# KTC-Security-Circle/3d-matching

Hardware: AMD Instinct MI355X
Metric: ICP iterations/sec + RANSAC hypotheses/sec, 100k↔100k pts, 1/2/4/8 GPU (higher is better)
Workload: dtype fp16-split MFMA NN screen + fp32 scan, exact fp64 NN decision, fp64 terms/solve; 1 GPU; cfg1: 100000<->100000 synthetic pair per GPU, 50 point-to-plane ICP iterations, brute-force NN (r=0.12), 1 GPU; ns=100000, nt_per_gpu=100000, parallelism=single, comm=none, comm_ranks=1

## Files before the change

### 3d-matching_amd/csrc/api.cpp

```cpp
#include <cfloat>
#include <chrono>
#include <hip/hip_runtime.h>
#include <string.h>

#include <algorithm>
#include <cmath>
#include <string>
#include <memory>
#include <mutex>
#include <unordered_map>
#include <vector>

#include "linalg.h"
#include "m3d_internal.h"
#include "ddmath.h"

using namespace m3d;

int m3d_fail(m3d_ctx* ctx, int code, const std::string& msg) {
  if (ctx) ctx->err = msg;
  return code;
}

KTimer::KTimer(m3d_ctx* c, int kid, hipStream_t s) : ctx(c), id(kid), st(s) {
// ... 1080 lines not shown
  for (Grid* g : c->grids) {
    grid_free(g);
    delete g;
  }
  for (auto& m : c->morton) {
    if (m.second->refs > 0)
      m.second->orphan = true;
    else
      m3d_cloud_destroy(m.second);
  }
  for (void** p : {reinterpret_cast<void**>(&c->slot), reinterpret_cast<void**>(&c->xyz64),
                   reinterpret_cast<void**>(&c->nrm64), reinterpret_cast<void**>(&c->xyz32)})
    if (in_block(*p, c->block, c->block_bytes)) *p = nullptr;
  block_release(c->block);
  hipFree(c->slot);
  hipFree(c->xyz64);
  hipFree(c->nrm64);
  hipFree(c->xyz32);
  block_release(c->rec64);
  delete c;
}

int64_t m3d_cloud_size(const m3d_cloud* c) { return c ? c->n : -1; }

namespace {
int ensure_grid(m3d_ctx* ctx, const m3d_cloud* c, double cell, hipStream_t st, const Grid** out) {
  for (Grid* g : c->grids)
    if (g->cell_req == cell && g->n_pts == c->n) {
      *out = g;
      return M3D_OK;
    }
  Grid* g = new Grid();
  float lohi[6];
  for (int k = 0; k < 3; ++k) {
    lohi[k] = c->lo[k];
    lohi[3 + k] = c->hi[k];
  }
  hipError_t e = grid_build(c->xyz32, c->n, cell, st, g, &ctx->tmp, c->has_bounds ? lohi : nullptr);
  if (e != hipSuccess) {
    grid_free(g);
    delete g;
    return m3d_fail(ctx, M3D_ERR_HIP, std::string("grid build: ") + hipGetErrorString(e));
  }
  g->cell_req = cell;
  c->grids.push_back(g);
  *out = g;
  return M3D_OK;
}

int ensure_morton_source(m3d_ctx* ctx, const m3d_cloud* c, double cell, const m3d_cloud** out,
                         const Grid** gout) {
  for (auto& m : c->morton)
    if (m.first == cell && m.second->n == c->n) {
      *out = m.second;
      *gout = m.second->grids.front();
      return M3D_OK;
    }
  m3d_cloud* mc = new m3d_cloud();
  mc->ctx = ctx;
  mc->ctx_id = ctx->id;
  Grid* g = new Grid();
  mc->grids.push_back(g);
  hipError_t e = morton_source(c, cell, mc, g, &ctx->tmp, nullptr);
  if (e != hipSuccess) {
    m3d_cloud_destroy(mc);
    return m3d_fail(ctx, M3D_ERR_HIP, std::string("morton source: ") + hipGetErrorString(e));
  }
  c->morton.emplace_back(cell, mc);
  constexpr size_t kMortonKeep = 4;
  for (size_t k = 0; c->morton.size() > kMortonKeep && k + 1 < c->morton.size();) {
    if (c->morton[k].second->refs == 0) {
      m3d_cloud_destroy(c->morton[k].second);
      c->morton.erase(c->morton.begin() + (ptrdiff_t)k);
    } else {
      ++k;
    }
  }
  *out = mc;
  *gout = g;
  return M3D_OK;
}

hipError_t enqueue_nn(m3d_icp* s, int64_t off, hipStream_t st, bool self_seed = false, int64_t q0 = 0,
                      int64_t q1 = -1) {
  m3d_ctx* ctx = s->ctx;
  const bool whole = q0 == 0 && (q1 < 0 || q1 == s->src->n);
  const bool seeded = self_seed && s->keys_clean && off == 0 && whole;
  s->keys_clean = false;
  if (s->params.nn_method == M3D_NN_GRID) {
    KTimer kt(ctx, M3D_KERNEL_NN, st);
    return launch_grid_nn(s->src->xyz32, s->src->n, s->sgrid, s->tgrid, off, s->state, s->keys,
                          s->near2, s->corr, s->dprev, s->tgt->xyz32, s->tgt->n, st, q0, q1,
                          s->hlist, s->hcnt, s->cand_cap, s->pcd64, s->tgt->xyz64, s->hcap, s->scan_xchunk);
  }
  if (!seeded) {
    hipError_t e = launch_icp_keyinit(s, off, st, q0, q1);
    if (e != hipSuccess) return e;
  }
  KTimer kt(ctx, M3D_KERNEL_NN, st);
  return launch_icp_nn(s, off, seeded, st, q0, q1);
}
}

extern "C++" {
namespace m3d {
int icp_shard_nn_range(m3d_icp* s, int64_t off, int64_t q0, int64_t q1, int64_t* dkeys, hipStream_t st) {
  hipError_t e = enqueue_nn(s, off, st, false, q0, q1);
  if (e == hipSuccess) e = launch_shard_winner(s, off, dkeys, st, q0, q1);
  if (e != hipSuccess) return m3d_fail(s->ctx, M3D_ERR_HIP, std::string("shard NN: ") + hipGetErrorString(e));
  return M3D_OK;
}
}
}

namespace {
int icp_create(m3d_ctx* ctx, const m3d_cloud* src, const m3d_cloud* tgt, double max_dist,
               const m3d_icp_params* params, m3d_icp** out, bool run_arena);
}

int m3d_icp_create(m3d_ctx* ctx, const m3d_cloud* src, const m3d_cloud* tgt, double max_dist,
                   const m3d_icp_params* params, m3d_icp** out) {
  return icp_create(ctx, src, tgt, max_dist, params, out, false);
}

namespace {
int32_t heavy_cap(const m3d_icp_params* params, int64_t coarse_max_occ) {
  constexpr int64_t kHeavyCell = 256;
  constexpr int32_t kHeavyCand = 256;
  static const int heavy_env = [] {
    const char* e = getenv("M3D_GRID_HEAVY");
    return e ? std::max(0, atoi(e)) : -1;
  }();
  if (params->nn_method != M3D_NN_GRID) return 0;
  return heavy_env > 0 ? heavy_env : (heavy_env < 0 && coarse_max_occ >= kHeavyCell ? kHeavyCand : 0);
}

int icp_create(m3d_ctx* ctx, const m3d_cloud* src, const m3d_cloud* tgt, double max_dist,
               const m3d_icp_params* params, m3d_icp** out, bool run_arena) {
  if (!ctx) return M3D_ERR_INVALID;
  CHECK_ARG(ctx, src && tgt && params && out, "invalid arguments");
  CHECK_ARG(ctx, max_dist > 0.0, "Invalid max_correspondence_distance.");
  CHECK_ARG(ctx, params->estimation == M3D_EST_POINT_TO_PLANE ||
                     params->estimation == M3D_EST_POINT_TO_POINT,
            "unknown estimation");
  CHECK_ARG(ctx, params->estimation != M3D_EST_POINT_TO_PLANE || tgt->nrm64 != nullptr || tgt->n == 0,
            "TransformationEstimationPointToPlane requires pre-computed normal vectors for target "
            "PointCloud.");
  CHECK_ARG(ctx, params->max_iteration >= 0, "max_iteration must be >= 0");
  CHECK_ARG(ctx, params->nn_method == M3D_NN_BRUTE || params->nn_method == M3D_NN_GRID,
            "unknown nn_method");
  hipSetDevice(ctx->device);
  const Grid *tg = nullptr, *sg = nullptr;
  const m3d_cloud* src_m = nullptr;
  int64_t coarse_max_occ = 0;
  int32_t cand_cap = 0;
  m3d_icp* s = new m3d_icp();
  {
    const double cell = max_dist * 1.001;
    int grc = ensure_grid(ctx, tgt, cell, nullptr, &tg);
    const m3d_cloud* ms = nullptr;
    if (!grc) grc = ensure_morton_source(ctx, src, cell, &ms, &sg);
    if (!grc) src_m = ms;
    if (!grc) {
      hipError_t e = ensure_target_rec(tgt, nullptr);
      if (e != hipSuccess) grc = m3d_fail(ctx, M3D_ERR_HIP, std::string("target records: ") + hipGetErrorString(e));
    }
    if (!grc && params->nn_method == M3D_NN_GRID) {
      hipError_t e = pin_ensure(ctx) == M3D_OK ? hipSuccess : hipErrorOutOfMemory;
      if (e == hipSuccess)
        e = grid_occupancy(const_cast<Grid*>(tg), &ctx->tmp, nullptr, pin_read<unsigned long long>(ctx, true),
                           pin_read<unsigned long long>(ctx, false));
      if (e != hipSuccess) grc = m3d_fail(ctx, M3D_ERR_HIP, std::string("grid occupancy: ") + hipGetErrorString(e));
    }
    if (!grc && params->nn_method == M3D_NN_GRID && tg->n_occ > 0) {
      coarse_max_occ = tg->max_occ;
      const double m = (double)tg->n_pts / (double)tg->n_occ;
      const int div = std::min(4, std::max(1, (int)std::floor(std::sqrt(m / 3.5))));
      if (div > 1) grc = ensure_grid(ctx, tgt, cell / div, nullptr, &tg);
    }
    if (!grc) {
      hipError_t e = build_grid_pts64(tgt, const_cast<Grid*>(tg), nullptr);
      if (e != hipSuccess) grc = m3d_fail(ctx, M3D_ERR_HIP, std::string("grid fp64 points: ") + hipGetErrorString(e));
    }
    if (!grc && params->nn_method == M3D_NN_BRUTE && tg->mf16 == nullptr) {
      hipError_t e = build_mfma_tiles(tgt, const_cast<Grid*>(tg), &ctx->tmp, nullptr);
      if (e != hipSuccess) grc = m3d_fail(ctx, M3D_ERR_HIP, std::string("mfma tiles: ") + hipGetErrorString(e));
    }
    if (!grc) {
      cand_cap = heavy_cap(params, coarse_max_occ);
      const size_t n1 = (size_t)std::max<int64_t>(src->n, 1);
      Carve cv;
      cv.add(&s->state, 1);
      if (params->nn_method == M3D_NN_BRUTE) nn_plan_shape(src->n, &s->nn_qblocks, &s->nn_budget);
      if (s->nn_qblocks > 0) {
        cv.add(&s->nn_cnt, (size_t)s->nn_qblocks);
        cv.add(&s->nn_seen, (size_t)s->nn_qblocks);
        cv.add(&s->nn_table, (size_t)s->nn_budget);
      }
      cv.add(&s->keys, n1);
      cv.add(&s->near2, n1);
      cv.add(&s->dprev, n1);
      cv.add(&s->ld64, n1);
      cv.add(&s->lidx, n1);
      cv.add(&s->corr, n1);
      if (params->nn_method == M3D_NN_BRUTE) cv.add(&s->seed, n1);
      cv.add(&s->partials, (size_t)(terms_blocks(src->n) * kTermSlots + kTermSlots));
      if (cand_cap > 0) {
        cv.add(&s->hlist, n1);
        cv.add(&s->hcnt, kDeferWords);
        s->hcap = (int32_t)n1;
      }
      cv.add(&s->pcd64, 3 * n1);
      size_t tot = 0;
      hipError_t e = run_arena ? ctx->run.reserve(cv.bytes()) : cv.alloc(&s->block, &tot, nullptr);
      if (e != hipSuccess) grc = m3d_fail(ctx, M3D_ERR_OOM, "device allocation failed (ICP loop arrays)");
      if (!grc && run_arena) cv.place(ctx->run.base);
    }
    if (!grc && s->hcnt != nullptr &&
        hipMemsetAsync(s->hcnt, 0, kDeferWords * sizeof(uint32_t), nullptr) != hipSuccess)
      grc = m3d_fail(ctx, M3D_ERR_HIP, "loop arrays: deferral counter");
    if (!grc && s->nn_cnt != nullptr &&
        hipMemsetAsync(s->nn_cnt, 0, (size_t)s->nn_qblocks * sizeof(uint32_t), nullptr) != hipSuccess)
      grc = m3d_fail(ctx, M3D_ERR_HIP, "loop arrays: NN plan counters");
    if (!grc) {
      hipError_t e = hipStreamSynchronize(nullptr);
      if (e != hipSuccess) grc = m3d_fail(ctx, M3D_ERR_HIP, std::string("loop setup: ") + hipGetErrorString(e));
    }
    if (grc) {
      block_release(s->block);
      delete s;
      return grc;
    }
  }
  s->ctx = ctx;
  s->ctx_id = ctx->id;
  s->src = src_m;
  src_m->refs += 1;
  s->user_src = src;
  s->tgt = tgt;
  s->params = *params;
  s->max_dist = max_dist;
  s->nblocks = terms_blocks(src->n);
  s->tgrid = tg;
  s->sgrid = sg;
  s->cand_cap = cand_cap;
  if (src->has_bounds && tgt->has_bounds)
    for (int k = 0; k < 3; ++k)
      if ((double)(tgt->hi[k] - tgt->lo[k]) * 2.0 < (double)(src->hi[k] - src->lo[k])) s->scan_xchunk = 8;
  s->sums = s->partials + s->nblocks * kTermSlots;
  *out = s;
  return M3D_OK;
}
}

void m3d_icp_destroy(m3d_icp* s) {
  if (!s) return;
  for (hipGraphExec_t g : s->graph)
    if (g != nullptr) hipGraphExecDestroy(g);
  if (s->cap_stream != nullptr) hipStreamDestroy(s->cap_stream);
  if (s->src != nullptr) {
    m3d_cloud* ms = const_cast<m3d_cloud*>(s->src);
    if (--ms->refs == 0 && ms->orphan) m3d_cloud_destroy(ms);
  }
  {
    ReleaseScope rs(s->ctx, s->ctx_id);
    block_release(s->block);
  }
  hipFree(s->xdk);
  hipFree(s->xcl);
  hipFree(s->xsums);
  delete s;
}

namespace {
bool eigen_is_identity(const double* T) {
  for (int i = 0; i < 4; ++i)
    for (int j = 0; j < 4; ++j) {
      const double a = T[4 * i + j];
      if (i == j ? !(std::fabs(a - 1.0) <= 1e-12 * std::min(std::fabs(a), 1.0)) : !(std::fabs(a) <= 1e-12))
        return false;
    }
  return true;
}

bool apply_init_of(const double* T, bool open3d_init) { return !(open3d_init && eigen_is_identity(T)); }

const double kIdentity16[16] = {1, 0, 0, 0, 0, 1, 0, 0, 0, 0, 1, 0, 0, 0, 0, 1};

int icp_reset(m3d_icp* s, const double* init, bool open3d_init, void* stream) {
  if (!s) return M3D_ERR_INVALID;
  Touch tch{s->ctx, S(stream)};
  m3d_ctx* ctx = s->ctx;
  const double* T = init ? init : kIdentity16;
  hipSetDevice(ctx->device);
  hipStream_t st = S(stream);
  HIPX(ctx, hipMemsetAsync(s->corr, 0xFF, sizeof(int32_t) * std::max<int64_t>(s->src->n, 1), st));
  HIPX(ctx, hipMemsetAsync(s->dprev, 0xFF, sizeof(int64_t) * std::max<int64_t>(s->src->n, 1), st));
  if (s->hcnt != nullptr) HIPX(ctx, hipMemsetAsync(s->hcnt, 0, kDeferWords * sizeof(uint32_t), st));
  HIPX(ctx, launch_icp_reset(s, T, apply_init_of(T, open3d_init), st));
  s->keys_clean = false;
  return M3D_OK;
}
}

int m3d_icp_reset(m3d_icp* s, const double* init, void* stream) { return icp_reset(s, init, true, stream); }

int m3d_icp_copy_points(const m3d_icp* s, double* dst, void* stream) {
  if (!s || (!dst && s->src->n > 0)) return M3D_ERR_INVALID;
  Touch tch{s->ctx, S(stream)};
  HIPX(s->ctx, launch_copy_points(s, dst, S(stream)));
  return M3D_OK;
}

namespace {
bool fused_tail(const m3d_icp* s, bool keys_back) {
  static const bool env = [] {
    const char* e = getenv("M3D_ICP_FUSED");
    return !(e && atoi(e) == 0);
  }();
  return env && (keys_back || s->nblocks <= 256);
}
}

int m3d_icp_step(m3d_icp* s, void* stream) {
  if (!s) return M3D_ERR_INVALID;
  Touch tch{s->ctx, S(stream)};
  m3d_ctx* ctx = s->ctx;
  hipStream_t st = S(stream);
  const bool reset = s->params.nn_method != M3D_NN_GRID && s->src->n > 0;
  const bool fused = fused_tail(s, reset);
  HIPX(ctx, enqueue_nn(s, 0, st, fused));
  if (fused) {
    KTimer kt(ctx, M3D_KERNEL_TERMS, st);
    HIPX(ctx, launch_icp_terms_solve(s, reset, st));
    s->keys_clean = reset;
    return M3D_OK;
  }
  { KTimer kt(ctx, M3D_KERNEL_TERMS, st); HIPX(ctx, launch_icp_terms_mode(s, 0, nullptr, nullptr, st)); }
  HIPX(ctx, launch_icp_reduce_solve(s, st));
  return M3D_OK;
}

namespace {
bool icp_graphs_on() {
  static const bool on = [] {
    const char* e = getenv("M3D_ICP_GRAPH");
    return !(e && atoi(e) == 0);
  }();
  return on;
}

int capture_steps(m3d_icp* s, int32_t n) {
  if (s->cap_stream == nullptr &&
      hipStreamCreateWithFlags(&s->cap_stream, hipStreamNonBlocking) != hipSuccess) {
    s->cap_stream = nullptr;
    return M3D_ERR_HIP;
  }
  const bool kc0 = s->keys_clean;
  const int slot = kc0 ? 1 : 0;
  if (hipStreamBeginCapture(s->cap_stream, hipStreamCaptureModeThreadLocal) != hipSuccess)
    return M3D_ERR_HIP;
  int rc = M3D_OK;
  for (int32_t k = 0; k < n && rc == M3D_OK; ++k) rc = m3d_icp_step(s, s->cap_stream);
  hipGraph_t g = nullptr;
  const hipError_t ee = hipStreamEndCapture(s->cap_stream, &g);
  const bool kc1 = s->keys_clean;
  s->keys_clean = kc0;
  hipGraphExec_t ex = nullptr;
  if (rc == M3D_OK && ee == hipSuccess && g != nullptr &&
      hipGraphInstantiate(&ex, g, nullptr, nullptr, 0) == hipSuccess) {
    if (s->graph[slot] != nullptr) hipGraphExecDestroy(s->graph[slot]);
    s->graph[slot] = ex;
    s->graph_n[slot] = n;
    s->graph_kc_out[slot] = kc1;
  } else {
    rc = rc ? rc : M3D_ERR_HIP;
  }
  if (g != nullptr) hipGraphDestroy(g);
  (void)hipGetLastError();
  return rc;
}
}

int m3d_icp_prepare_steps(m3d_icp* s, int32_t n) {
  if (!s) return M3D_ERR_INVALID;
  CHECK_ARG(s->ctx, n >= 0, "n must be >= 0");
  if (n < 2 || !icp_graphs_on() || s->graph_off) return M3D_OK;
  hipSetDevice(s->ctx->device);
  if (capture_steps(s, n) != M3D_OK) {
    s->graph_off = true;
    (void)hipGetLastError();
  }
  return M3D_OK;
}

int m3d_icp_steps(m3d_icp* s, int32_t n, void* stream) {
  if (!s) return M3D_ERR_INVALID;
  Touch tch{s->ctx, S(stream)};
  CHECK_ARG(s->ctx, n >= 0, "n must be >= 0");
  if (n >= 2 && icp_graphs_on() && !s->graph_off && !s->ctx->profiling) {
    const int slot = s->keys_clean ? 1 : 0;
    const bool have = s->graph[slot] != nullptr && s->graph_n[slot] == n;
    const bool again = s->seen_n[slot] == n;
    s->seen_n[slot] = n;
    if (!have && again) {
      hipSetDevice(s->ctx->device);
      if (capture_steps(s, n) != M3D_OK) s->graph_off = true;
    }
    if ((have || again) && !s->graph_off) {
      HIPX(s->ctx, hipGraphLaunch(s->graph[slot], S(stream)));
      s->keys_clean = s->graph_kc_out[slot];
      return M3D_OK;
    }
// ... 1608 lines not shown
  std::lock_guard<std::mutex> lk(g_bc_mu);
  int n = 0;
  for (const CachedBlock& b : g_bc) {
    if (b.dev != cur) continue;
    if (hipMemset(b.p, byte & 0xFF, b.bytes) != hipSuccess) return M3D_ERR_HIP;
    ++n;
  }
  if (hipDeviceSynchronize() != hipSuccess) return M3D_ERR_HIP;
  return n;
}

int m3d_debug_icp_defer_count(m3d_icp* s, uint32_t count, void* stream) {
  if (!s) return M3D_ERR_INVALID;
  CHECK_ARG(s->ctx, s->hcnt != nullptr, "this loop has no deferral list (grid NN with a candidate cap only)");
  Touch tch{s->ctx, S(stream)};
  HIPX(s->ctx, hipMemcpyAsync(s->hcnt, &count, sizeof(count), hipMemcpyHostToDevice, S(stream)));
  HIPX(s->ctx, hipStreamSynchronize(S(stream)));
  return M3D_OK;
}

int m3d_debug_nn_plan_host(const uint32_t* counts, int64_t n, int64_t budget, int64_t smax, int64_t ntiles,
                           uint32_t* out) {
  if (!counts || !out || smax < 1 || ntiles < 1) return M3D_ERR_INVALID;
  const uint32_t tau = plan_host(counts, n, budget, smax, ntiles, nullptr, out);
  return tau == 0 ? M3D_ERR_INVALID : (int)tau;
}

int m3d_debug_icp_nn_plan(m3d_icp* s, const int32_t* S_, int64_t n, void* stream) {
  if (!s || !S_) return M3D_ERR_INVALID;
  CHECK_ARG(s->ctx, s->nn_qblocks > 0 && nn_plan_on(), "this loop's NN launch takes no plan");
  CHECK_ARG(s->ctx, n == s->nn_qblocks, "one S per query block of 512 sources");
  const int64_t ntiles = s->tgrid->mf_npad / 1024;
  std::vector<uint32_t> Sv((size_t)n), table((size_t)s->nn_budget);
  int64_t sum = 0;
  for (int64_t x = 0; x < n; ++x) {
    CHECK_ARG(s->ctx, S_[x] >= 1 && S_[x] <= ntiles && S_[x] <= 255, "S out of range [1, min(ntiles, 255)]");
    Sv[(size_t)x] = (uint32_t)S_[x];
    sum += S_[x];
  }
  CHECK_ARG(s->ctx, sum <= s->nn_budget, "more slices than resident block slots");
  plan_table_of(Sv.data(), n, s->nn_budget, table.data());
  Touch tch{s->ctx, S(stream)};
  const int32_t forced = 2;
  HIPX(s->ctx, hipMemcpyAsync(s->nn_table, table.data(), sizeof(uint32_t) * table.size(), hipMemcpyHostToDevice, S(stream)));
  HIPX(s->ctx, hipMemcpyAsync(&s->state->plan_ok, &forced, sizeof(forced), hipMemcpyHostToDevice, S(stream)));
  HIPX(s->ctx, hipStreamSynchronize(S(stream)));
  return M3D_OK;
}

int m3d_debug_icp_nn_plan_read(m3d_icp* s, uint32_t* counts, uint32_t* table, int32_t* shape3, void* stream) {
  if (!s || !shape3) return M3D_ERR_INVALID;
  shape3[0] = s->nn_qblocks;
  shape3[1] = s->nn_budget;
  shape3[2] = 0;
  if (s->nn_qblocks <= 0) return M3D_OK;
  Touch tch{s->ctx, S(stream)};
  if (counts)
    HIPX(s->ctx, hipMemcpyAsync(counts, s->nn_seen, sizeof(uint32_t) * (size_t)s->nn_qblocks, hipMemcpyDeviceToHost, S(stream)));
  if (table)
    HIPX(s->ctx, hipMemcpyAsync(table, s->nn_table, sizeof(uint32_t) * (size_t)s->nn_budget, hipMemcpyDeviceToHost, S(stream)));
  HIPX(s->ctx, hipMemcpyAsync(&shape3[2], &s->state->plan_ok, sizeof(int32_t), hipMemcpyDeviceToHost, S(stream)));
  HIPX(s->ctx, hipStreamSynchronize(S(stream)));
  return M3D_OK;
}

int m3d_debug_icp_seed_read(m3d_icp* s, float* seed, int32_t* corr, float* tgt32, int32_t* info2, void* stream) {
  if (!s || !info2) return M3D_ERR_INVALID;
  CHECK_ARG(s->ctx, s->seed != nullptr && s->tgt->rec64 != nullptr,
            "this loop keeps no seed records (brute-force NN on a non-empty target only)");
  info2[0] = s->keys_clean ? 1 : 0;
  Touch tch{s->ctx, S(stream)};
  HIPX(s->ctx, hipMemcpyAsync(&info2[1], &s->state->mfma_ok, sizeof(int32_t), hipMemcpyDeviceToHost, S(stream)));
  const size_t ns = (size_t)s->src->n, nt = (size_t)s->tgt->n;
  if (seed && ns > 0)
    HIPX(s->ctx, hipMemcpyAsync(seed, s->seed, sizeof(float4) * ns, hipMemcpyDeviceToHost, S(stream)));
  if (corr && ns > 0)
    HIPX(s->ctx, hipMemcpyAsync(corr, s->corr, sizeof(int32_t) * ns, hipMemcpyDeviceToHost, S(stream)));
  if (tgt32)
    HIPX(s->ctx, hipMemcpyAsync(tgt32, s->tgt->xyz32, sizeof(float4) * nt, hipMemcpyDeviceToHost, S(stream)));
  HIPX(s->ctx, hipStreamSynchronize(S(stream)));
  return M3D_OK;
}

}
```

### 3d-matching_amd/csrc/icp.hip

```cpp
#include <float.h>

#include <algorithm>
#include <string>
#include <type_traits>
#include <vector>
#include <stdlib.h>

#include "lds_dma.h"
#include "linalg.h"
#include "m3d_internal.h"
#include "nnkey.h"

namespace m3d {

constexpr int kTermsBlock = 512;
constexpr double kU = 5.9604644775390625e-08;
constexpr double kU64 = 1.1102230246251565e-16;


__device__ __forceinline__ float f32_ru(double d) {
  const float f = (float)d;
  const uint32_t u = __float_as_uint(f);
  const uint32_t up = f == 0.0f ? 1u : ((int32_t)u >= 0 ? u + 1u : u - 1u);
  return (double)f < d ? __uint_as_float(up) : f;
}

__device__ void refresh_rt32_from(IcpState* s, const double* T, double r2, double r, const FrameParams& f,
                                  int iters) {
  const double* cs = f.cs;
  const double* ct = f.ct;
  const double pinf = f.pinf, qinf = f.qinf;
  double rowl1 = 0.0, tinf = 0.0;
  for (int i = 0; i < 3; ++i) {
    const double* r = T + 4 * i;
    const double tp = fma(r[2], cs[2], fma(r[1], cs[1], r[0] * cs[0])) + r[3] - ct[i];
    for (int j = 0; j < 3; ++j) s->Rt32[3 * i + j] = (float)r[j];
    s->Rt32[9 + i] = (float)tp;
    rowl1 = fmax(rowl1, fabs(r[0]) + fabs(r[1]) + fabs(r[2]));
    tinf = fmax(tinf, fabs(tp));
  }
  double tabs = 0.0, csinf = 0.0, ctinf = 0.0;
  for (int i = 0; i < 3; ++i) {
    tabs = fmax(tabs, fabs(T[4 * i + 3]));
    csinf = fmax(csinf, fabs(cs[i]));
    ctinf = fmax(ctinf, fabs(ct[i]));
  }
  const double mag = rowl1 * (csinf + pinf) + tabs + ctinf + qinf;
  const double E32 = 1.01 * kU * (5.0 * rowl1 * pinf + 4.0 * tinf + qinf);
  const double E = E32 + 8.0 * kU64 * 1.7320508075688772 * (double)(iters + 2) * mag + 1e-11 * (mag + 1.0);
  const double eq = 1.7320508075688772 * E * 1.01;
  const float eqf = f32_ru(eq), bef = f32_ru(2.0 * eq * 1.01);
  s->eq = isfinite(eqf) ? eqf : FLT_MAX;
  s->band_e = isfinite(bef) ? bef : FLT_MAX;
  const double e = 2.0 * (3.0 * kU * (r + 1.7320508075688772 * E) * (r + 1.7320508075688772 * E) +
                          2.0 * 1.7320508075688772 * E * r + 3.0 * E * E);
  float hi = f32_ru(r2 + e);
  if (!isfinite(hi)) hi = FLT_MAX;
  s->r2_hi = hi;
  const double Q = rowl1 * pinf + tinf;
  const double E1 = 5.0 * kU * (3.0 * qinf * qinf + 6.0 * Q * qinf);
  const double es = 2.0 * (E1 + 6.0 * kU * (double)hi + 12.0 * kU * Q * Q) + 1e-30;
  const float esf = f32_ru(es);
  s->screen_eps = isfinite(esf) ? esf : FLT_MAX;
  const double S = f.s16;
  const double As = 2.0 * Q * S, Ts = qinf * S;
  const double Ws = 3.0 * Ts * Ts * (1.0 + 1e-6);
  const double u16 = 4.8828125e-04, sig = 2.98023223876953125e-08;
  const double P = 3.0 * As * Ts;
  const double Esplit = 3.0 * u16 * u16 * P + 4.0 * sig * 3.0 * (As + Ts) + u16 * u16 * Ws + 2.0 * sig;
  const double Eacc = 32.0 * kU * 1.01 * (P + Ws);
  const double E1m = 1.05 * (Esplit + Eacc) / (S * S) + kU * 3.0 * qinf * qinf;
  const double esm = 2.0 * (E1m + 6.0 * kU * (double)hi + 12.0 * kU * Q * Q) + 1e-30;
  const float esmf = f32_ru(esm);
  s->screen_eps_m = isfinite(esmf) ? esmf : FLT_MAX;
  s->mfma_scale = (float)S;
  s->mfma_ok = (As < 16384.0 && Ts < 16384.0 && Ws < 16384.0 && isfinite(esmf) &&
                hi < FLT_MAX && esmf < 0.25f * FLT_MAX) ? 1 : 0;
}

__device__ void refresh_rt32(IcpState* s, const FrameParams& f) {
  double T[16];
  for (int k = 0; k < 16; ++k) T[k] = s->T[k];
  refresh_rt32_from(s, T, s->r2, sqrt(s->r2), f, s->iters);
}

__device__ __forceinline__ void set_identity(double* M) {
  for (int k = 0; k < 16; ++k) M[k] = (k % 5 == 0) ? 1.0 : 0.0;
}

__device__ __forceinline__ void reset_eval(IcpState* s, double r2, const FrameParams& f) {
  s->fitness = s->rmse = s->prev_fitness = s->prev_rmse = 0.0;
  s->count = 0;
  s->evals = s->iters = s->done = s->converged = 0;
  s->ticket = 0;
  s->plan_ok = 0;
  s->r2 = r2;
  s->bound_ok = 0;
  refresh_rt32(s, f);
  s->eq_prev = s->eq;
}

__global__ void icp_init_kernel(IcpState* s, double T0, double T1, double T2, double T3, double T4,
                                double T5, double T6, double T7, double T8, double T9, double T10,
                                double T11, double r2, FrameParams f, int apply_init) {
  if (threadIdx.x != 0) return;
  const double T[12] = {T0, T1, T2, T3, T4, T5, T6, T7, T8, T9, T10, T11};
  for (int k = 0; k < 12; ++k) s->T[k] = T[k];
  s->T[12] = s->T[13] = s->T[14] = 0.0;
  s->T[15] = 1.0;
  for (int k = 0; k < 16; ++k) s->dT[k] = apply_init ? s->T[k] : ((k % 5 == 0) ? 1.0 : 0.0);
  set_identity(s->last_upd);
  reset_eval(s, r2, f);
}

__global__ void icp_set_T_kernel(IcpState* s, const double* __restrict__ T, double r2, FrameParams f) {
  if (threadIdx.x != 0) return;
  for (int k = 0; k < 16; ++k) s->T[k] = s->dT[k] = T[k];
  set_identity(s->last_upd);
  reset_eval(s, r2, f);
}

__global__ __launch_bounds__(64) void val_states_kernel(IcpState* __restrict__ states,
                                                        const double* __restrict__ T,
                                                        const int32_t* __restrict__ list, int64_t n,
                                                        double r2, FrameParams f) {
  const int64_t k = (int64_t)blockIdx.x * 64 + threadIdx.x;
  if (k >= n) return;
  IcpState* s = states + k;
  const double* Th = T + 16 * (int64_t)list[k];
  for (int j = 0; j < 16; ++j) s->T[j] = s->dT[j] = Th[j];
  reset_eval(s, r2, f);
}

__global__ __launch_bounds__(256) void keyinit_kernel(const float4* __restrict__ src32, int64_t ns,
                                                      const float4* __restrict__ tgt32,
                                                      int64_t nt_shard, int64_t off,
                                                      const IcpState* __restrict__ s,
                                                      const int32_t* __restrict__ prev,
                                                      const int64_t* __restrict__ dprev,
                                                      int64_t* __restrict__ keys,
                                                      uint32_t* __restrict__ near2, int64_t q0) {
  if (s->done) return;
  const int64_t i = q0 + (int64_t)blockIdx.x * 256 + threadIdx.x;
  if (i >= ns) return;
  const float* Rt = s->Rt32;
  const float4 p = src32[i];
  float x, y, z;
  xform32(Rt, p, x, y, z);
  keys[i] = seed_key(s, i, p, x, y, z, tgt32, nt_shard, off, prev, dprev);
  near2[i] = kNearNone;
}

template <bool k32>
__device__ __forceinline__ double swap_add(double a, double b) {
  const uint64_t ua = (uint64_t)__double_as_longlong(a), ub = (uint64_t)__double_as_longlong(b);
  const uint32_t alo = (uint32_t)ua, ahi = (uint32_t)(ua >> 32);
  const uint32_t blo = (uint32_t)ub, bhi = (uint32_t)(ub >> 32);
  const auto rl = k32 ? __builtin_amdgcn_permlane32_swap(alo, blo, false, false)
                      : __builtin_amdgcn_permlane16_swap(alo, blo, false, false);
  const auto rh = k32 ? __builtin_amdgcn_permlane32_swap(ahi, bhi, false, false)
                      : __builtin_amdgcn_permlane16_swap(ahi, bhi, false, false);
  const double na = __longlong_as_double((long long)(((uint64_t)rh[0] << 32) | rl[0]));
  const double nb = __longlong_as_double((long long)(((uint64_t)rh[1] << 32) | rl[1]));
  return na + nb;
}

template <int kOff>
__device__ __forceinline__ double xchg_add(double a, double b, int lane) {
  const bool hi = (lane & kOff) != 0;
  const double keep = hi ? b : a, send = hi ? a : b;
  return keep + xor_lane_f64(send, kOff);
}

__device__ __forceinline__ double wave_transpose_sum32(const double (&v)[32], int lane) {
  double w16[16], w8[8], w4[4], w2[2];
#pragma unroll
  for (int j = 0; j < 16; ++j) w16[j] = swap_add<true>(v[j], v[j + 16]);
#pragma unroll
  for (int j = 0; j < 8; ++j) w8[j] = swap_add<false>(w16[j], w16[j + 8]);
#pragma unroll
  for (int j = 0; j < 4; ++j) w4[j] = xchg_add<8>(w8[j], w8[j + 4], lane);
#pragma unroll
  for (int j = 0; j < 2; ++j) w2[j] = xchg_add<4>(w4[j], w4[j + 2], lane);
  const double w1 = xchg_add<2>(w2[0], w2[1], lane);
  return w1 + xor_lane_f64(w1, 1);
}

template <int kEst>
__device__ __forceinline__ void terms_add(double (&acc)[30], const double (&Q)[3], const double (&q)[3],
                                          const double (&n)[3], double d2, const double (&c)[3]) {
  const double d[3] = {Q[0] - q[0], Q[1] - q[1], Q[2] - q[2]};
  acc[28] += 1.0;
  acc[29] += d2;
  if (kEst == M3D_EST_POINT_TO_PLANE) {
    const double r = d[0] * n[0] + d[1] * n[1] + d[2] * n[2];
    double J[6];
    cross3(Q, n, J);
    J[3] = n[0];
    J[4] = n[1];
    J[5] = n[2];
    int k = 0;
#pragma unroll
    for (int x = 0; x < 6; ++x)
#pragma unroll
      for (int y = x; y < 6; ++y) acc[k++] += J[x] * J[y];
#pragma unroll
    for (int x = 0; x < 6; ++x) acc[21 + x] += J[x] * r;
    acc[27] += r * r;
  } else {
    const double pc[3] = {Q[0] - c[0], Q[1] - c[1], Q[2] - c[2]};
    const double qc[3] = {q[0] - c[0], q[1] - c[1], q[2] - c[2]};
#pragma unroll
    for (int x = 0; x < 3; ++x) {
      acc[x] += pc[x];
      acc[3 + x] += qc[x];
#pragma unroll
      for (int y = 0; y < 3; ++y) acc[6 + 3 * x + y] += pc[x] * qc[y];
    }
  }
}

struct TermsArgs {
  double* pcd64;
  const float4* src32;
  int64_t ns;
  const double* tgt64;
  const double* nrm64;
  const double* rec64;
  int64_t nt_shard, off;
  const int64_t* keys;
  uint32_t* near2;
  GridDev g;
  const int32_t* claim;
  const int64_t* dmin;
  int64_t* dprev;
  int32_t* corr;
  int est;
  double c[3];
  int64_t* reset_keys;
  float4* seed;
};

#if M3D_TAIL_CLOCK
__device__ unsigned long long g_tail_clock[3 * 4096 + 24];
#endif
#if M3D_TERMS_CLOCK
__device__ unsigned long long g_terms_clock[4096 * 8];
#define M3D_TPH(k)                               \
  do {                                           \
    __builtin_amdgcn_s_waitcnt(0);               \
    tph_[k] = __builtin_amdgcn_s_memrealtime();  \
  } while (0)
#else
#define M3D_TPH(k) \
  do {             \
  } while (0)
#endif
template <bool kWT, int kEst>
__device__ __forceinline__ void terms_block(const TermsArgs& a, const IcpState* __restrict__ s,
                                            double* __restrict__ partials) {
  __shared__ double red[kTermSlots][kTermsBlock / kWave];
#if M3D_TERMS_CLOCK
  unsigned long long tph_[8];
#endif
  M3D_TPH(0);
  double acc[30];
#pragma unroll
  for (int k = 0; k < 30; ++k) acc[k] = 0.0;
  constexpr int kP = 1;
  int64_t ii[kP];
  bool valid[kP];
  double vs[kP][3];
  int64_t gj[kP];
  double d2[kP];
  bool fixed[kP];
  uint64_t k1[kP];
  float n2[kP];
#pragma unroll
  for (int u = 0; u < kP; ++u) {
    const int64_t i = ((int64_t)blockIdx.x * kP + u) * kTermsBlock + threadIdx.x;
    valid[u] = i < a.ns;
    ii[u] = valid[u] ? i : 0;
    gj[u] = -1;
    d2[u] = 0.0;
    fixed[u] = true;
    if (a.claim == nullptr) {
      k1[u] = valid[u] ? (uint64_t)a.keys[ii[u]] : (uint64_t)kKeyNone;
      n2[u] = valid[u] ? __uint_as_float(a.near2[ii[u]]) : kInf;
    } else if (valid[u]) {
      const int32_t cj = a.claim[ii[u]];
      const int64_t dm = a.dmin[ii[u]];
      if (cj != 0x7FFFFFFF) {
        gj[u] = cj;
        d2[u] = __longlong_as_double(dm);
      }
      if (a.dprev != nullptr) a.dprev[ii[u]] = dm;
    }
    q64_of(s->dT, a.pcd64 + 3 * ii[u], vs[u]);
    if (valid[u])
      for (int k = 0; k < 3; ++k) a.pcd64[3 * ii[u] + k] = vs[u][k];
  }
  M3D_TPH(1);
  if (a.claim == nullptr) {
    bool amb[kP];
    float X[kP], qx[kP], qy[kP], qz[kP];
    int64_t bj[kP];
    double bd[kP];
#pragma unroll
    for (int u = 0; u < kP; ++u) {
      if (valid[u] && a.reset_keys != nullptr) {
        a.reset_keys[ii[u]] = kKeyNone;
        a.near2[ii[u]] = kNearNone;
      }
      X[u] = valid[u] && k1[u] != (uint64_t)kKeyNone ? search_bound(key_d2(k1[u]), s->band_e, s->r2_hi) : -1.0f;
      amb[u] = X[u] >= 0.0f && n2[u] <= X[u];
#if M3D_TAIL_CLOCK
      {
        const int64_t gw = (int64_t)blockIdx.x * (kTermsBlock / kWave) + threadIdx.x / kWave;
        const int na = __popcll(__ballot(amb[u]));
        if ((threadIdx.x & (kWave - 1)) == 0 && gw < 4096) g_tail_clock[2 * 4096 + 8 + gw] = na;
      }
#endif
      qx[u] = qy[u] = qz[u] = 0.0f;
      if (amb[u]) xform32(s->Rt32, a.src32[ii[u]], qx[u], qy[u], qz[u]);
      bj[u] = -1;
      bd[u] = 0.0;
    }
    resolve_wave(amb[0], a.g, a.tgt64, a.off, qx[0], qy[0], qz[0], X[0], vs[0], s->r2, bj[0], bd[0]);
#pragma unroll
    for (int u = 0; u < kP; ++u) {
      if (amb[u]) {
        gj[u] = bj[u];
        d2[u] = bd[u];
      } else if (valid[u] && key_real(k1[u])) {
        const int64_t c = (int64_t)(uint32_t)k1[u];
        if (c >= a.off && c < a.off + a.nt_shard) {
          gj[u] = c;
          fixed[u] = false;
        }
      }
    }
  }
  M3D_TPH(2);
  double tq[kP][3], tn[kP][3];
  double pad[kP][2];
#pragma unroll
  for (int u = 0; u < kP; ++u) {
    pad[u][0] = pad[u][1] = 0.0;
    const bool own = valid[u] && gj[u] >= a.off && gj[u] < a.off + a.nt_shard;
    const int64_t l = own ? gj[u] - a.off : 0;
    if (a.nt_shard == 0) {
      for (int k = 0; k < 3; ++k) tq[u][k] = tn[u][k] = 0.0;
    } else if (a.rec64 != nullptr) {
      const double4 r0 = reinterpret_cast<const double4*>(a.rec64)[2 * l];
      const double4 r1 = reinterpret_cast<const double4*>(a.rec64)[2 * l + 1];
      tq[u][0] = r0.x;
      tq[u][1] = r0.y;
      tq[u][2] = r0.z;
      tn[u][0] = r0.w;
      tn[u][1] = r1.x;
      tn[u][2] = r1.y;
      pad[u][0] = r1.z;
      pad[u][1] = r1.w;
    } else {
#pragma unroll
      for (int k = 0; k < 3; ++k) {
        tq[u][k] = a.tgt64[3 * l + k];
        tn[u][k] = kEst == M3D_EST_POINT_TO_PLANE ? a.nrm64[3 * l + k] : 0.0;
      }
    }
  }
  M3D_TPH(3);
#pragma unroll
  for (int u = 0; u < kP; ++u) {
    if (!valid[u]) continue;
    if (!fixed[u]) {
      const double d = d2_64(vs[u], tq[u]);
      if (d < s->r2) {
        d2[u] = d;
      } else {
        gj[u] = -1;
      }
    }
    const int64_t i = ii[u];
    if (a.corr != nullptr) a.corr[i] = (int32_t)gj[u];
    if (kWT && a.seed != nullptr) {
      a.seed[i] = make_float4(__int_as_float(__double2loint(pad[u][0])), __int_as_float(__double2hiint(pad[u][0])),
                              __int_as_float(__double2loint(pad[u][1])), __int_as_float((int32_t)gj[u]));
    }
    if (gj[u] < a.off || gj[u] >= a.off + a.nt_shard) continue;
    terms_add<kEst>(acc, vs[u], tq[u], tn[u], d2[u], a.c);
  }
  M3D_TPH(4);
  const int lane = threadIdx.x & (kWave - 1), wave = threadIdx.x / kWave;
  {
    double v[32];
#pragma unroll
    for (int k = 0; k < 32; ++k) v[k] = k < 30 ? acc[k] : 0.0;
    const double w = wave_transpose_sum32(v, lane);
    if ((lane & 1) == 0) red[lane >> 1][wave] = w;
  }
  M3D_TPH(5);
  __syncthreads();
  M3D_TPH(6);
  if (threadIdx.x < kTermSlots) {
    double v = 0.0;
    if (threadIdx.x < 30)
      for (int w = 0; w < kTermsBlock / kWave; ++w) v += red[threadIdx.x][w];
    double* dst = partials + (int64_t)blockIdx.x * kTermSlots + threadIdx.x;
    if (kWT)
      __hip_atomic_store(reinterpret_cast<unsigned long long*>(dst), __double_as_longlong(v),
                         __ATOMIC_RELAXED, __HIP_MEMORY_SCOPE_AGENT);
    else
      *dst = v;
  }
  M3D_TPH(7);
#if M3D_TERMS_CLOCK
  {
    const int64_t gw = (int64_t)blockIdx.x * (kTermsBlock / kWave) + threadIdx.x / kWave;
    if ((threadIdx.x & (kWave - 1)) == 0 && gw < 4096)
      for (int k = 0; k < 8; ++k) g_terms_clock[8 * gw + k] = tph_[k];
  }
#endif
}

template <int kEst>
__global__ __launch_bounds__(kTermsBlock) void terms_kernel(TermsArgs a, const IcpState* __restrict__ s,
                                                            double* __restrict__ partials) {
  if (s->done) return;
  terms_block<false, kEst>(a, s, partials);
}

__global__ __launch_bounds__(256) void shard_winner_kernel(
    const double* __restrict__ pcd64, const float4* __restrict__ src32, int64_t ns,
    const double* __restrict__ tgt64, int64_t nt_shard, int64_t off, GridDev g,
    const IcpState* __restrict__ s, const int64_t* __restrict__ keys,
    const uint32_t* __restrict__ near2, int32_t* __restrict__ lidx, int64_t* __restrict__ ld64,
    int64_t* __restrict__ dkey, int64_t q0) {
  if (s->done) return;
  const int64_t i0 = q0 + (int64_t)blockIdx.x * 256 + threadIdx.x;
  const bool valid = i0 < ns;
  const int64_t i = valid ? i0 : 0;
  const uint64_t k1 = valid ? (uint64_t)keys[i] : (uint64_t)kKeyNone;
  const bool need = k1 != (uint64_t)kKeyNone;
  double Q[3] = {0.0, 0.0, 0.0};
  if (need) q64_of(s->dT, pcd64 + 3 * i, Q);
  const float4 p32 = need ? src32[i] : make_float4(0.0f, 0.0f, 0.0f, 0.0f);
  int64_t gj;
  double d;
  winner_fp64(valid, k1, need ? __uint_as_float(near2[i]) : kInf, s, g, tgt64, off, nt_shard, p32, Q, gj, d);
  if (!valid) return;
  const int64_t k = gj >= 0 ? __double_as_longlong(d) : kKeyNone;
  lidx[i] = (int32_t)gj;
  ld64[i] = k;
  dkey[i] = k;
}

__global__ __launch_bounds__(256) void shard_claim_kernel(int64_t ns, const IcpState* __restrict__ s,
                                                          const int32_t* __restrict__ lidx,
                                                          const int64_t* __restrict__ ld64,
                                                          const int64_t* __restrict__ dmin,
                                                          int32_t* __restrict__ claim) {
  if (s->done) return;
  const int64_t i = (int64_t)blockIdx.x * 256 + threadIdx.x;
  if (i >= ns) return;
  claim[i] = (lidx[i] >= 0 && ld64[i] == dmin[i]) ? lidx[i] : 0x7FFFFFFF;
}

constexpr int kReduceGroups = 32;
template <int kSlots>
__device__ __forceinline__ double group_sum(const double* __restrict__ partials, int64_t nblocks,
                                            int g, int slot) {
  double v = 0.0;
#pragma unroll 4
  for (int64_t b = g; b < nblocks; b += kReduceGroups) v += partials[b * kSlots + slot];
  return v;
}

template <int kSlots>
__global__ __launch_bounds__(kReduceGroups * kSlots) void reduce_kernel(
    const double* __restrict__ partials, int64_t nblocks, double* __restrict__ sums,
    const IcpState* __restrict__ s, const uint32_t* __restrict__ hcnt) {
  if (s != nullptr && s->done) return;
  __shared__ double red[kReduceGroups][kSlots];
  const int slot = threadIdx.x & (kSlots - 1);
  const int g = threadIdx.x / kSlots;
  red[g][slot] = group_sum<kSlots>(partials, nblocks, g, slot);
  __syncthreads();
  if (threadIdx.x < kSlots) {
    double t = 0.0;
    for (int k = 0; k < kReduceGroups; ++k) t += red[k][threadIdx.x];
    if (hcnt != nullptr && threadIdx.x == kSlots - 2) t = (double)hcnt[0];
    if (hcnt != nullptr && threadIdx.x == kSlots - 1) t = (double)hcnt[kDeferFault];
    sums[threadIdx.x] = t;
  }
}

struct SolveParams {
  double rel_fit, rel_rmse;
  int max_iter, est;
  int64_t ns;
  double c[3];
  FrameParams f;
};

struct SolveIn {
  int32_t evals, iters;
  double prev_fit, prev_rmse, r2;
  float eq;
  double T[16];
  float rt[12];
};

// ... 163 lines not shown
  for (int k = 0; k < kReduceGroups; ++k)
    tot += __longlong_as_double(__hip_atomic_load(
        reinterpret_cast<unsigned long long*>(partials + (int64_t)k * kTermSlots + slot), __ATOMIC_RELAXED,
        __HIP_MEMORY_SCOPE_AGENT));
  sums[slot] = tot;
  __shared__ double out[kTermSlots];
  out[slot] = tot;
  __syncthreads();
  if (slot == 0) s->ticket = 0;
  if (do_solve) solve_state<kEst>(out, s, sp, in);
}

constexpr int kPlanPer = kPlanMaxQ / kWave;
struct PlanIn {
  uint32_t t[kPlanPer];
  int32_t flag;
};
__device__ __forceinline__ void plan_in(const PlanArgs& pa, const IcpState* s, int lane, PlanIn& in) {
  in.flag = __hip_atomic_load(&s->plan_ok, __ATOMIC_RELAXED, __HIP_MEMORY_SCOPE_AGENT);
#pragma unroll
  for (int k = 0; k < kPlanPer; ++k) {
    const int x = k * kWave + lane;
    in.t[k] = __hip_atomic_load(&pa.cnt[min(x, pa.n - 1)], __ATOMIC_RELAXED, __HIP_MEMORY_SCOPE_AGENT);
  }
#pragma unroll
  for (int k = 0; k < kPlanPer; ++k) in.t[k] = k * kWave + lane < pa.n ? min(in.t[k], kPlanTmax) : 0u;
}
template <bool kMax>
__device__ __forceinline__ uint32_t plan_wave_red(uint32_t v) {
  const auto op = [](uint32_t a, uint32_t b) { return kMax ? max(a, b) : a + b; };
#pragma unroll
  for (int o = 1; o < 16; o <<= 1) v = op(v, (uint32_t)xor_lane((int)v, o, kWave));
  const auto rl = [&](int l) { return (uint32_t)__builtin_amdgcn_readlane((int)v, l); };
  return op(op(rl(0), rl(16)), op(rl(32), rl(48)));
}
__device__ void plan_wave(const PlanArgs& pa, IcpState* s, int lane, const PlanIn& in) {
  uint32_t tmax = 0, tsum = 0;
#pragma unroll
  for (int k = 0; k < kPlanPer; ++k) {
    const int x = k * kWave + lane;
    if (x < pa.n) {
      pa.cnt[x] = 0u;
      pa.seen[x] = in.t[k];
    }
    tmax = max(tmax, in.t[k]);
    tsum += in.t[k];
  }
  if (in.flag == 2) return;
  tmax = plan_wave_red<true>(tmax);
  tsum = plan_wave_red<false>(tsum);
  const uint32_t cap = (uint32_t)pa.cap;
  const uint32_t tau = plan_tau(tmax, tsum, (uint32_t)pa.n, (uint32_t)pa.budget, [&](uint32_t m) {
    uint32_t a = 0;
#pragma unroll
    for (int k = 0; k < kPlanPer; ++k)
      if (k * kWave < pa.n)
        a += k * kWave + lane < pa.n ? plan_slices(in.t[k], m, cap) : 0u;
    return plan_wave_red<false>(a);
  });
  uint32_t S[kPlanPer];
#pragma unroll
  for (int k = 0; k < kPlanPer; ++k) S[k] = k * kWave + lane < pa.n ? plan_slices(in.t[k], tau, cap) : 0u;
  int pos = 0;
  for (uint32_t y = 0; y < cap; ++y) {
    const int pos0 = pos;
#pragma unroll
    for (int k = 0; k < kPlanPer; ++k) {
      if (k * kWave >= pa.n) break;
      const bool has = S[k] > y;
      const uint64_t m = __ballot(has);
      const int at = pos + (int)__builtin_amdgcn_mbcnt_hi((uint32_t)(m >> 32), __builtin_amdgcn_mbcnt_lo((uint32_t)m, 0u));
      if (has && at < pa.budget) pa.table[at] = plan_entry((uint32_t)(k * kWave + lane), y, S[k]);
      pos += __builtin_popcountll(m);
    }
    if (pos == pos0) break;
  }
  for (int i = pos + lane; i < pa.budget; i += kWave) pa.table[i] = kPlanEmpty;
  if (lane == 0) s->plan_ok = 1;
}

struct PlanNone {
  static constexpr int32_t n = 0;
};
template <int kEst, bool kPlanner>
__global__ __launch_bounds__(kTermsBlock) void terms_solve_kernel(
    TermsArgs a, IcpState* s, double* partials, int64_t nblocks, double* __restrict__ sums,
    SolveParams sp, int do_solve, std::conditional_t<kPlanner, PlanArgs, PlanNone> pa) {
  if (s->done) return;
#if M3D_TAIL_CLOCK
  const unsigned long long clk0 = __builtin_amdgcn_s_memrealtime();
#endif
  terms_block<true, kEst>(a, s, partials);
#if M3D_TAIL_CLOCK
  {
    const unsigned long long clk1 = __builtin_amdgcn_s_memrealtime();
    const int64_t gw = (int64_t)blockIdx.x * (kTermsBlock / kWave) + threadIdx.x / kWave;
    if ((threadIdx.x & (kWave - 1)) == 0 && gw < 4096) {
      g_tail_clock[2 * gw] = clk0;
      g_tail_clock[2 * gw + 1] = clk1;
    }
  }
#endif
  __shared__ double red[kReduceGroups][kTermSlots];
  __shared__ int last;
  asm volatile("s_waitcnt vmcnt(0)" ::: "memory");
  __syncthreads();
  if (threadIdx.x == 0) {
    const uint32_t t =
        __hip_atomic_fetch_add(&s->ticket, 1u, __ATOMIC_RELAXED, __HIP_MEMORY_SCOPE_AGENT);
    last = (t == (uint32_t)(nblocks - 1));
  }
  __syncthreads();
  if (!last) return;
  M3D_TCLK(0);
  SolveIn in;
  if (do_solve && threadIdx.x < kWave) solve_in(s, in);
  const bool planner = kPlanner && pa.n > 0 && threadIdx.x >= kWave && threadIdx.x < 2 * kWave;
  PlanIn pin;
  if constexpr (kPlanner)
    if (planner) plan_in(pa, s, threadIdx.x - kWave, pin);
  const int slot = threadIdx.x & (kTermSlots - 1);
  constexpr int kG = kReduceGroups / (kTermsBlock / kTermSlots);
  double gv[kG];
#pragma unroll
  for (int u = 0; u < kG; ++u) gv[u] = 0.0;
  const int g0 = threadIdx.x / kTermSlots;
  constexpr int kR = 8;
  for (int64_t b0 = 0; b0 < nblocks; b0 += kR * kReduceGroups) {
    double t[kR][kG];
#pragma unroll
    for (int r = 0; r < kR; ++r)
#pragma unroll
      for (int u = 0; u < kG; ++u) {
        const int64_t b = b0 + r * kReduceGroups + g0 + u * (kTermsBlock / kTermSlots);
        t[r][u] = b < nblocks
                      ? __longlong_as_double(__hip_atomic_load(
                            reinterpret_cast<unsigned long long*>(partials + b * kTermSlots + slot),
                            __ATOMIC_RELAXED, __HIP_MEMORY_SCOPE_AGENT))
                      : 0.0;
      }
#pragma unroll
    for (int r = 0; r < kR; ++r)
#pragma unroll
      for (int u = 0; u < kG; ++u) gv[u] += t[r][u];
  }
  M3D_TCLK(8);
#pragma unroll
  for (int u = 0; u < kG; ++u) red[g0 + u * (kTermsBlock / kTermSlots)][slot] = gv[u];
  __syncthreads();
  if (threadIdx.x < kTermSlots) {
    double t = 0.0;
    for (int k = 0; k < kReduceGroups; ++k) t += red[k][threadIdx.x];
    red[0][threadIdx.x] = t;
    sums[threadIdx.x] = t;
  }
  M3D_TCLK(9);
  __syncthreads();
  M3D_TCLK(1);
  if (threadIdx.x < kWave) {
    if (threadIdx.x == 0) s->ticket = 0;
    if (do_solve) solve_state<kEst>(red[0], s, sp, in);
  } else if (planner) {
    if constexpr (kPlanner) plan_wave(pa, s, threadIdx.x - kWave, pin);
  }
  M3D_TCLK(2);
}

__global__ __launch_bounds__(256) void nn_finalize_kernel(const double* __restrict__ pcd64,
                                                          const float4* __restrict__ src32,
                                                          int64_t ns,
                                                          const double* __restrict__ tgt64,
                                                          int64_t nt, GridDev g,
                                                          const IcpState* __restrict__ s,
                                                          const int64_t* __restrict__ keys,
                                                          const uint32_t* __restrict__ near2,
                                                          const int32_t* __restrict__ slot,
                                                          int32_t* __restrict__ idx,
                                                          double* __restrict__ d2out) {
  const SlotWinner w = slot_winner((int64_t)blockIdx.x * 256 + threadIdx.x, pcd64, src32, ns, tgt64, nt, g, s, keys,
                                   near2);
  if (!w.valid) return;
  const int64_t o = slot != nullptr ? (int64_t)slot[w.i] : w.i;
  idx[o] = (int32_t)w.gj;
  if (d2out != nullptr) d2out[o] = w.gj >= 0 ? w.d : INFINITY;
}

template <typename V, bool kGather>
__global__ void permute_kernel(const V* __restrict__ v, const int32_t* __restrict__ slot, int64_t n,
                               V* __restrict__ dst) {
  const int64_t k = (int64_t)blockIdx.x * 256 + threadIdx.x;
  if (k >= n) return;
  if (kGather)
    dst[k] = v[slot[k]];
  else
    dst[slot[k]] = v[k];
}

constexpr int kPairChunk = 1024;

__global__ __launch_bounds__(256) void pair_count_kernel(const int32_t* __restrict__ v, int64_t n,
                                                         int32_t* __restrict__ cnt) {
  __shared__ int part[4];
  const int64_t base = (int64_t)blockIdx.x * kPairChunk;
  int c = 0;
#pragma unroll
  for (int u = 0; u < 4; ++u) {
    const int64_t i = base + u * 256 + threadIdx.x;
    c += __popcll(__ballot(i < n && v[i] >= 0));
  }
  if ((threadIdx.x & (kWave - 1)) == 0) part[threadIdx.x / kWave] = c;
  __syncthreads();
  if (threadIdx.x == 0) cnt[blockIdx.x] = part[0] + part[1] + part[2] + part[3];
}

__global__ __launch_bounds__(1024) void pair_scan_kernel(int32_t* __restrict__ cnt, int64_t nb) {
  __shared__ int32_t wsum[16];
  __shared__ int32_t carry_s;
  const int lane = threadIdx.x & (kWave - 1), w = threadIdx.x / kWave;
  if (threadIdx.x == 0) carry_s = 0;
  __syncthreads();
  for (int64_t b0 = 0; b0 < nb; b0 += 1024) {
    const int64_t b = b0 + threadIdx.x;
    const int32_t x = b < nb ? cnt[b] : 0;
    int32_t incl = x;
#pragma unroll
    for (int o = 1; o < kWave; o <<= 1) {
      const int32_t y = __shfl_up(incl, o, kWave);
      if (lane >= o) incl += y;
    }
    if (lane == kWave - 1) wsum[w] = incl;
    __syncthreads();
    int32_t before = carry_s;
    for (int k = 0; k < w; ++k) before += wsum[k];
    if (b < nb) cnt[b] = before + incl - x;
    __syncthreads();
    if (threadIdx.x == 1023) carry_s = before + incl;
    __syncthreads();
  }
  if (threadIdx.x == 0) cnt[nb] = carry_s;
}

__global__ __launch_bounds__(256) void pair_place_kernel(const int32_t* __restrict__ v, int64_t n,
                                                         const int32_t* __restrict__ off,
                                                         int32_t* __restrict__ pairs) {
  __shared__ int grp[16];
  const int lane = threadIdx.x & (kWave - 1), w = threadIdx.x / kWave;
  const int64_t base = (int64_t)blockIdx.x * kPairChunk;
  bool hit[4];
  int32_t val[4];
  uint64_t m[4];
#pragma unroll
  for (int u = 0; u < 4; ++u) {
    const int64_t i = base + u * 256 + threadIdx.x;
    val[u] = i < n ? v[i] : -1;
    hit[u] = val[u] >= 0;
    m[u] = __ballot(hit[u]);
    if (lane == 0) grp[u * 4 + w] = __popcll(m[u]);
  }
  __syncthreads();
  const uint64_t below = lane == 0 ? 0ull : (~0ull >> (64 - lane));
  int32_t o = off[blockIdx.x];
#pragma unroll
  for (int u = 0; u < 4; ++u) {
    int32_t before = o;
    for (int k = 0; k < w; ++k) before += grp[u * 4 + k];
    if (hit[u]) {
      const int32_t k = before + __popcll(m[u] & below);
      pairs[2 * (int64_t)k] = (int32_t)(base + u * 256 + threadIdx.x);
      pairs[2 * (int64_t)k + 1] = val[u];
    }
    for (int k = 0; k < 4; ++k) o += grp[u * 4 + k];
  }
}

__global__ void keys_to_idx_kernel(const int64_t* __restrict__ keys, int64_t n,
                                   int32_t* __restrict__ idx) {
  const int64_t i = (int64_t)blockIdx.x * 256 + threadIdx.x;
  if (i < n) idx[i] = keys[i] == kKeyNone ? -1 : (int32_t)(uint32_t)keys[i];
}

static FrameParams frame_of(const m3d_icp* s) {
  FrameParams f;
  for (int k = 0; k < 3; ++k) {
    f.cs[k] = s->src->center[k];
    f.ct[k] = s->tgt->center[k];
  }
  f.pinf = s->src->rmax;
  f.qinf = s->tgt->rmax;
  f.s16 = s->tgt->s16;
  f.shared = s->tgt->center_given;
  return f;
}

static SolveParams solve_params(const m3d_icp* s) {
  SolveParams sp;
  sp.rel_fit = s->params.relative_fitness;
  sp.rel_rmse = s->params.relative_rmse;
  sp.max_iter = s->params.max_iteration;
  sp.est = s->params.estimation;
  sp.ns = s->ns_total > 0 ? s->ns_total : s->src->n;
  for (int k = 0; k < 3; ++k) sp.c[k] = s->src->center[k];
  sp.f = frame_of(s);
  return sp;
}

template <typename F>
static void with_est(int est, F f) {
  if (est == M3D_EST_POINT_TO_PLANE)
    f(std::integral_constant<int, M3D_EST_POINT_TO_PLANE>{});
  else
    f(std::integral_constant<int, M3D_EST_POINT_TO_POINT>{});
}

static hipError_t reset_points(const m3d_icp* s, hipStream_t st) {
  if (s->src->n == 0) return hipSuccess;
  return hipMemcpyAsync(s->pcd64, s->src->xyz64, sizeof(double) * 3 * s->src->n, hipMemcpyDeviceToDevice, st);
}

static hipError_t reset_plan_counts(const m3d_icp* s, hipStream_t st) {
  if (s->nn_cnt == nullptr) return hipSuccess;
  return hipMemsetAsync(s->nn_cnt, 0, (size_t)s->nn_qblocks * sizeof(uint32_t), st);
}

hipError_t launch_icp_state_init(IcpState* state, const double* T, bool apply_init, double r2, const FrameParams& f,
                                 hipStream_t st) {
  icp_init_kernel<<<1, 64, 0, st>>>(state, T[0], T[1], T[2], T[3], T[4], T[5], T[6], T[7], T[8], T[9], T[10], T[11],
                                    r2, f, apply_init ? 1 : 0);
  return hipGetLastError();
}

hipError_t launch_icp_reset(const m3d_icp* s, const double* T, bool apply_init, hipStream_t st) {
  hipError_t e = reset_points(s, st);
  if (e == hipSuccess) e = reset_plan_counts(s, st);
  if (e != hipSuccess) return e;
  return launch_icp_state_init(s->state, T, apply_init, s->max_dist * s->max_dist, frame_of(s), st);
}

hipError_t launch_icp_set_T(const m3d_icp* s, const double* T_dev, hipStream_t st) {
  hipError_t e = reset_points(s, st);
  if (e == hipSuccess) e = reset_plan_counts(s, st);
  if (e != hipSuccess) return e;
  icp_set_T_kernel<<<1, 64, 0, st>>>(s->state, T_dev, s->max_dist * s->max_dist, frame_of(s));
  return hipGetLastError();
}

__global__ void copy_points_kernel(const IcpState* __restrict__ s, const double* __restrict__ v,
                                   const int32_t* __restrict__ slot, int64_t n, double* __restrict__ dst) {
  const int64_t k = (int64_t)blockIdx.x * 256 + threadIdx.x;
  if (k >= n) return;
  const int64_t o = (int64_t)slot[k];
  bool apply = s->evals == 0;
  if (apply) {
    bool eye = true;
    for (int e = 0; e < 16; ++e) eye = eye && s->dT[e] == ((e % 5) == 0 ? 1.0 : 0.0);
    apply = !eye;
  }
  if (apply) {
    double q[3];
    q64_of(s->dT, v + 3 * k, q);
    for (int c = 0; c < 3; ++c) dst[3 * o + c] = q[c];
  } else {
    for (int c = 0; c < 3; ++c) dst[3 * o + c] = v[3 * k + c];
  }
}

hipError_t launch_copy_points(const m3d_icp* s, double* dst, hipStream_t st) {
  const int64_t n = s->src->n;
  if (n == 0) return hipSuccess;
  copy_points_kernel<<<(unsigned)((n + 255) / 256), 256, 0, st>>>(s->state, s->pcd64, s->src->slot, n, dst);
  return hipGetLastError();
}

hipError_t launch_val_states(const m3d_icp* s, const double* T_dev, const int32_t* list, int64_t n,
                             IcpState* states, hipStream_t st) {
  if (n == 0) return hipSuccess;
  val_states_kernel<<<(unsigned)((n + 63) / 64), 64, 0, st>>>(states, T_dev, list, n,
                                                              s->max_dist * s->max_dist, frame_of(s));
  return hipGetLastError();
}

hipError_t launch_icp_keyinit(const m3d_icp* s, int64_t off, hipStream_t st, int64_t q0, int64_t q1) {
  const int64_t ns = q1 < 0 ? s->src->n : q1;
  if (ns <= q0) return hipSuccess;
  keyinit_kernel<<<(unsigned)((ns - q0 + 255) / 256), 256, 0, st>>>(
      s->src->xyz32, ns, s->tgt->xyz32, s->tgt->n, off, s->state, s->corr, s->dprev, s->keys,
      s->near2, q0);
  return hipGetLastError();
}


__global__ __launch_bounds__(256) void pack_rec_kernel(const double* __restrict__ xyz,
                                                       const double* __restrict__ nrm,
                                                       const float4* __restrict__ xyz32, int64_t n,
                                                       double* __restrict__ rec) {
  const int64_t i = (int64_t)blockIdx.x * 256 + threadIdx.x;
  if (i >= n) return;
  double r[8];
  for (int k = 0; k < 3; ++k) {
    r[k] = xyz[3 * i + k];
    r[3 + k] = nrm != nullptr ? nrm[3 * i + k] : 0.0;
  }
  const float4 p = xyz32[i];
  r[6] = __hiloint2double(__float_as_int(p.y), __float_as_int(p.x));
  r[7] = __hiloint2double(__float_as_int(p.w), __float_as_int(p.z));
// ... 90 lines not shown
                         const uint32_t* hcnt, hipStream_t st) {
  if (slots == 16)
    reduce_kernel<16><<<1, kReduceGroups * 16, 0, st>>>(partials, rows, out, s, hcnt);
  else if (slots == kTermSlots)
    reduce_kernel<kTermSlots><<<1, kReduceGroups * kTermSlots, 0, st>>>(partials, rows, out, s, hcnt);
  else
    return hipErrorInvalidValue;
  return hipGetLastError();
}

hipError_t launch_icp_reduce(const m3d_icp* s, double* sums, hipStream_t st) {
  if (s->nblocks <= 256) return launch_reduce(s->partials, s->nblocks, kTermSlots, sums, s->state, nullptr, st);
  launch_reduce_groups(s, sums, 0, st);
  return hipGetLastError();
}

hipError_t launch_icp_reduce_solve(const m3d_icp* s, hipStream_t st) {
  if (s->nblocks <= 256) {
    hipError_t e = launch_icp_reduce(s, s->sums, st);
    return e == hipSuccess ? launch_icp_solve(s, s->sums, st) : e;
  }
  launch_reduce_groups(s, s->sums, 1, st);
  return hipGetLastError();
}

static void launch_terms_solve(const TermsArgs& ta, const m3d_icp* s, double* sums, int do_solve,
                               hipStream_t st) {
  const unsigned nb = (unsigned)s->nblocks;
  const SolveParams sp = solve_params(s);
  const PlanArgs pa = nn_plan_args(s);
  with_est(ta.est, [&](auto e) {
    if (pa.n > 0)
      terms_solve_kernel<decltype(e)::value, true><<<nb, kTermsBlock, 0, st>>>(ta, s->state, s->partials, s->nblocks,
                                                                               sums, sp, do_solve, pa);
    else
      terms_solve_kernel<decltype(e)::value, false><<<nb, kTermsBlock, 0, st>>>(ta, s->state, s->partials, s->nblocks,
                                                                                sums, sp, do_solve, PlanNone{});
  });
}

hipError_t launch_icp_terms_reduce(const m3d_icp* s, int64_t off, const int32_t* claim,
                                   const int64_t* dmin, double* sums, bool reset_keys,
                                   hipStream_t st) {
  const int64_t ns = s->src->n;
  if (ns == 0) {
    hipError_t e = launch_icp_terms_mode(s, off, claim, dmin, st);
    return e == hipSuccess ? launch_icp_reduce(s, sums, st) : e;
  }
  launch_terms_solve(terms_args(s, off, claim, dmin, reset_keys), s, sums, 0, st);
  return hipGetLastError();
}

hipError_t launch_icp_solve_state(IcpState* state, const double* sums, double relative_fitness, double relative_rmse,
                                  int32_t max_iteration, int32_t estimation, int64_t ns, const double* center,
                                  const FrameParams& f, hipStream_t st) {
  SolveParams sp;
  sp.rel_fit = relative_fitness;
  sp.rel_rmse = relative_rmse;
  sp.max_iter = max_iteration;
  sp.est = estimation;
  sp.ns = ns;
  for (int k = 0; k < 3; ++k) sp.c[k] = center[k];
  sp.f = f;
  with_est(sp.est, [&](auto e) { solve_kernel<decltype(e)::value><<<1, 64, 0, st>>>(sums, state, sp); });
  return hipGetLastError();
}

hipError_t launch_icp_solve(const m3d_icp* s, const double* sums, hipStream_t st) {
  const SolveParams sp = solve_params(s);
  return launch_icp_solve_state(s->state, sums, sp.rel_fit, sp.rel_rmse, sp.max_iter, sp.est, sp.ns, sp.c, sp.f, st);
}

hipError_t launch_icp_terms_solve(const m3d_icp* s, bool reset_keys, hipStream_t st) {
  const int64_t ns = s->src->n;
  if (ns == 0) {
    hipError_t e = launch_icp_terms_mode(s, 0, nullptr, nullptr, st);
    if (e == hipSuccess) e = launch_icp_reduce(s, s->sums, st);
    return e == hipSuccess ? launch_icp_solve(s, s->sums, st) : e;
  }
  launch_terms_solve(terms_args(s, 0, nullptr, nullptr, reset_keys), s, s->sums, 1, st);
  return hipGetLastError();
}

hipError_t launch_nn_finalize(const m3d_icp* s, int32_t* idx, double* d2, hipStream_t st) {
  const int64_t ns = s->src->n;
  if (ns == 0) return hipSuccess;
  nn_finalize_kernel<<<(unsigned)((ns + 255) / 256), 256, 0, st>>>(
      s->pcd64, s->src->xyz32, ns, s->tgt->xyz64, s->tgt->n, s->tgrid->dev, s->state, s->keys,
      s->near2, s->src->slot, idx, d2);
  return hipGetLastError();
}

template <typename V, bool kGather>
static hipError_t launch_permute(const V* v, const int32_t* slot, int64_t n, V* dst, hipStream_t st) {
  if (n == 0) return hipSuccess;
  permute_kernel<V, kGather><<<(unsigned)((n + 255) / 256), 256, 0, st>>>(v, slot, n, dst);
  return hipGetLastError();
}

hipError_t launch_scatter_i32(const int32_t* v, const int32_t* slot, int64_t n, int32_t* dst,
                              hipStream_t st) {
  if (n > 0 && slot == nullptr) return hipMemcpyAsync(dst, v, sizeof(int32_t) * n, hipMemcpyDeviceToDevice, st);
  return launch_permute<int32_t, false>(v, slot, n, dst, st);
}
hipError_t launch_gather_i32(const int32_t* v, const int32_t* slot, int64_t n, int32_t* dst, hipStream_t st) {
  return launch_permute<int32_t, true>(v, slot, n, dst, st);
}
hipError_t launch_scatter_f64(const double* v, const int32_t* slot, int64_t n, double* dst, hipStream_t st) {
  return launch_permute<double, false>(v, slot, n, dst, st);
}

hipError_t launch_corr_pairs(const int32_t* v, int64_t n, int32_t* cnt, int32_t* pairs, hipStream_t st) {
  if (n <= 0) return hipMemsetAsync(cnt, 0, sizeof(int32_t), st);
  const int64_t nb = (n + kPairChunk - 1) / kPairChunk;
  pair_count_kernel<<<(unsigned)nb, 256, 0, st>>>(v, n, cnt);
  pair_scan_kernel<<<1, 1024, 0, st>>>(cnt, nb);
  pair_place_kernel<<<(unsigned)nb, 256, 0, st>>>(v, n, cnt, pairs);
  return hipGetLastError();
}

hipError_t launch_shard_winner(const m3d_icp* s, int64_t off, int64_t* dkey, hipStream_t st,
                               int64_t q0, int64_t q1) {
  const int64_t ns = q1 < 0 ? s->src->n : q1;
  if (ns <= q0) return hipSuccess;
  shard_winner_kernel<<<(unsigned)((ns - q0 + 255) / 256), 256, 0, st>>>(
      s->pcd64, s->src->xyz32, ns, s->tgt->xyz64, s->tgt->n, off, s->tgrid->dev, s->state,
      s->keys, s->near2, s->lidx, s->ld64, dkey, q0);
  return hipGetLastError();
}

hipError_t launch_shard_claim(const m3d_icp* s, const int64_t* dmin, int32_t* claim, hipStream_t st) {
  const int64_t ns = s->src->n;
  if (ns == 0) return hipSuccess;
  shard_claim_kernel<<<(unsigned)((ns + 255) / 256), 256, 0, st>>>(ns, s->state, s->lidx, s->ld64,
                                                                   dmin, claim);
  return hipGetLastError();
}

hipError_t launch_keys_to_idx(const int64_t* keys, int64_t n, int32_t* idx, hipStream_t st) {
  if (n == 0) return hipSuccess;
  keys_to_idx_kernel<<<(unsigned)((n + 255) / 256), 256, 0, st>>>(keys, n, idx);
  return hipGetLastError();
}

int64_t terms_blocks(int64_t ns) { return ns > 0 ? (ns + kTermsBlock - 1) / kTermsBlock : 1; }

}

#if M3D_TERMS_CLOCK
extern "C" int m3d_debug_terms_clock(unsigned long long* out, int n) {
  return hipMemcpyFromSymbol(out, HIP_SYMBOL(m3d::g_terms_clock), sizeof(unsigned long long) * (size_t)n) == hipSuccess ? 0 : -1;
}
#endif
#if M3D_TAIL_CLOCK
extern "C" int m3d_debug_tail_clock(unsigned long long* out, int n) {
  return hipMemcpyFromSymbol(out, HIP_SYMBOL(m3d::g_tail_clock), sizeof(unsigned long long) * (size_t)n) == hipSuccess ? 0 : -1;
}
#endif
```

### 3d-matching_amd/csrc/m3d_internal.h

```cpp
#pragma once

#include <hip/hip_runtime.h>
#include <stdint.h>

#include <algorithm>
#include <string>
#include <utility>
#include <functional>
#include <memory>
#include <mutex>
#include <vector>

#include "../../include/m3d.h"
#include "nn_plan.h"

#define M3D_CONST __attribute__((address_space(4)))

namespace m3d {

constexpr int kWave = 64;

__device__ __forceinline__ double wave_sum(double v) {
#pragma unroll
  for (int o = kWave / 2; o > 0; o >>= 1) v += __shfl_xor(v, o);
// ... 231 lines not shown
  m3d_ctx* ctx = nullptr;
  int64_t nc = 0, nc_pad = 0;
  double* p64 = nullptr;
  double* q64 = nullptr;
  float4* p32 = nullptr;
  float4* q32 = nullptr;
  double cs[3] = {0, 0, 0}, ct[3] = {0, 0, 0};
  double pmax2 = 0.0;
  double qmaxinf = 0.0;
  uint4* ca16 = nullptr;
  double s16 = 0.0;
};

struct m3d_cloud {
  m3d_ctx* ctx = nullptr;
  uint64_t ctx_id = 0;
  int64_t n = 0, n_pad = 0;
  double* xyz64 = nullptr;
  double* nrm64 = nullptr;
  float4* xyz32 = nullptr;
  double center[3] = {0, 0, 0};
  double rmax = 0.0;
  float lo[3] = {0, 0, 0}, hi[3] = {0, 0, 0};
  bool has_bounds = false;
  double s16 = 1.0;
  int center_given = 0;
  mutable std::vector<m3d::Grid*> grids;
  mutable double* rec64 = nullptr;
  mutable std::vector<std::pair<double, m3d_cloud*>> morton;
  int32_t* slot = nullptr;
  mutable int refs = 0;
  bool orphan = false;
  void* block = nullptr;
  size_t block_bytes = 0;
};

struct m3d_mesh {
  m3d_ctx* ctx = nullptr;
  uint64_t ctx_id = 0;
  int64_t nv = 0, nf = 0;
  int64_t usable = 0;
  double* v64 = nullptr;
  int32_t* tri = nullptr;
  double* tri9 = nullptr;
  uint8_t* ok = nullptr;
  void* block = nullptr;
  size_t block_bytes = 0;
  double lo[3] = {0, 0, 0}, hi[3] = {0, 0, 0};
  bool grid_built = false;
  m3d::TriGridDev grid{};
  void* gblock = nullptr;
  size_t gblock_bytes = 0;
  int64_t nrefs = 0;
  int32_t doublings = 0;
  int32_t last_rounds = 0;
};

struct m3d_icp {
  m3d_ctx* ctx = nullptr;
  uint64_t ctx_id = 0;
  const m3d_cloud* src = nullptr;
  const m3d_cloud* user_src = nullptr;
  const m3d_cloud* tgt = nullptr;
  m3d_icp_params params{};
  double max_dist = 0.0;
  void* block = nullptr;
  m3d::IcpState* state = nullptr;
  int64_t* keys = nullptr;
  uint32_t* near2 = nullptr;
  int64_t* dprev = nullptr;
  int64_t* ld64 = nullptr;
  int32_t* lidx = nullptr;
  int32_t* hlist = nullptr;
  uint32_t* hcnt = nullptr;
  int32_t hcap = 0;
  int32_t cand_cap = 0;
  int32_t scan_xchunk = 0;
  bool keys_clean = false;
  uint32_t* nn_cnt = nullptr;
  uint32_t* nn_seen = nullptr;
  uint32_t* nn_table = nullptr;
  int32_t nn_qblocks = 0;
  int32_t nn_budget = 0;
  int32_t* corr = nullptr;
  float4* seed = nullptr;
  double* pcd64 = nullptr;
  double* partials = nullptr;
  double* sums = nullptr;
  int64_t nblocks = 0;
  const m3d::Grid* sgrid = nullptr;
  const m3d::Grid* tgrid = nullptr;
  int64_t ns_total = 0;
  bool xready_tgt = false;
  bool xready_src = false;
  int64_t* xdk = nullptr;
  int32_t* xcl = nullptr;
  double* xsums = nullptr;
  hipStream_t cap_stream = nullptr;
  hipGraphExec_t graph[2] = {nullptr, nullptr};
  int32_t graph_n[2] = {-1, -1};
  bool graph_kc_out[2] = {false, false};
  int32_t seen_n[2] = {-1, -1};
  bool graph_off = false;
};

int m3d_fail(m3d_ctx* ctx, int code, const std::string& msg);

struct KTimer {
  m3d_ctx* ctx;
  int id;
  hipStream_t st;
  hipEvent_t end = nullptr;
  KTimer(m3d_ctx* c, int kid, hipStream_t s);
  ~KTimer();
};
#define M3D_HIP_CHECK(ctx, expr)                                                        \
  do {                                                                                  \
    hipError_t e_ = (expr);                                                             \
    if (e_ != hipSuccess)                                                               \
      return m3d_fail((ctx), M3D_ERR_HIP, std::string(#expr) + ": " + hipGetErrorString(e_)); \
  } while (0)

namespace m3d {
hipError_t launch_pack_corr(const double* src, const double* tgt, const int32_t* corr, int64_t nc,
                            const double* p_src, const double* p_tgt, double* p64, double* q64,
                            hipStream_t st);
hipError_t launch_sum3(const double* a, int64_t n, double* partial , int blocks,
                       hipStream_t st);
hipError_t launch_center_pack(const double* a, int64_t n, int64_t n_pad, const double c[3],
                              float4* out, float pad_value, float* maxnorm_partial, int blocks,
                              int maxinf, hipStream_t st);
hipError_t launch_cloud_pack(const double* a, int64_t n, int64_t n_pad, const double* sum_part,
                             int sum_blocks, double* cdev, const double c[3], float4* out, float pad_value,
                             float* part7, int blocks, double* pin_c ,
                             float* pin7 , hipStream_t st);
struct ScoreMf;
struct ScoreFuse {
  const ScoreMf* mf;
  double thr;
  int mode;
};
hipError_t launch_kabsch3(const m3d_corrset* cs, const int32_t* triples, uint64_t seed,
                          int64_t hyp0, int64_t H, double thr_sq, double* T_out, uint8_t* status,
                          HypF32* hypf, const int32_t* done, ZeroArgs z, hipStream_t st,
                          const ScoreFuse* fuse = nullptr);
hipError_t ensure_target_rec(const m3d_cloud* c, hipStream_t st);
hipError_t build_grid_pts64(const m3d_cloud* c, Grid* g, hipStream_t st);
hipError_t launch_kabsch3_one(const m3d_corrset* cs, const int32_t* tri, double* T_out,
                              int32_t* status, hipStream_t st);
int64_t count_one_blocks(int64_t nc);
hipError_t launch_count_one(const m3d_corrset* cs, const double* T, double thr, int mode,
                            int32_t* partials, int64_t max_blocks, uint32_t* ticket, int64_t* out,
                            hipStream_t st);
hipError_t launch_hypf_from_T(const m3d_corrset* cs, const double* T, int64_t H, double thr_sq,
                              HypF32* hypf, ZeroArgs z, hipStream_t st);
struct ScoreMf {
  uint4* hb16 = nullptr;
  float* heps = nullptr;
  int64_t h_pad = 0;
};
int64_t score_mf_hpad(int64_t H);
hipError_t launch_corr16(m3d_corrset* cs, hipStream_t st);
hipError_t launch_score_prep(const m3d_corrset* cs, const double* T64, int64_t H, double thr,
                             int mode, const ScoreMf& mf, hipStream_t st);
hipError_t launch_score(const m3d_corrset* cs, const HypF32* hypf, int64_t H, int32_t* counts,
                        const double* T64, double thr, int mode, int64_t* stats,
                        const int32_t* done, const ScoreMf& mf, hipStream_t st);
hipError_t launch_select(const int32_t* counts, int64_t h_begin, int64_t n, int64_t nc,
                         int64_t max_iter, int early_stop, double es_thr, double es_conf,
                         const double* T_batch, RansacState* rs, hipStream_t st);
hipError_t launch_ransac_init(RansacState* rs, const int64_t* stats, int done, hipStream_t st);
hipError_t launch_copy_result(const RansacState* rs, int64_t nc, const int64_t* stats,
                              m3d_ransac_result* out_dev, hipStream_t st);
hipError_t launch_ransac_pack_key(const m3d_ransac_result* r, int64_t hyp0, int64_t* key,
                                  hipStream_t st);
hipError_t launch_ransac_shard_key(const m3d_ransac_result* r, int64_t hyp0, int64_t* buf,
                                   hipStream_t st);
hipError_t launch_ransac_shard_pack(const m3d_ransac_result* r, int64_t hyp0, int64_t* buf,
                                    hipStream_t st);
int icp_shard_nn_range(m3d_icp* s, int64_t off, int64_t q0, int64_t q1, int64_t* dkeys, hipStream_t st);
bool icp_nn_range_ok(const m3d_icp* s);

hipError_t launch_icp_keyinit(const m3d_icp* s, int64_t shard_offset, hipStream_t st, int64_t q0 = 0,
                              int64_t q1 = -1);
hipError_t launch_icp_nn(const m3d_icp* s, int64_t shard_offset, bool self_seed, hipStream_t st,
                         int64_t q0 = 0, int64_t q1 = -1);
int64_t nn_resident_slots();
bool nn_plan_on();
void nn_plan_shape(int64_t ns, int32_t* qblocks, int32_t* budget);
PlanArgs nn_plan_args(const m3d_icp* s);
hipError_t launch_icp_reset(const m3d_icp* s, const double* T, bool apply_init, hipStream_t st);
hipError_t launch_icp_state_init(IcpState* state, const double* T, bool apply_init, double r2, const FrameParams& f,
                                 hipStream_t st);
hipError_t launch_copy_points(const m3d_icp* s, double* dst, hipStream_t st);
hipError_t launch_icp_terms_solve(const m3d_icp* s, bool reset_keys, hipStream_t st);
hipError_t launch_nn_finalize(const m3d_icp* s, int32_t* idx, double* d2, hipStream_t st);
int64_t terms_blocks(int64_t ns);
hipError_t launch_reduce(const double* partials, int64_t rows, int slots, double* out, const IcpState* s,
                         const uint32_t* hcnt, hipStream_t st);
hipError_t launch_icp_reduce(const m3d_icp* s, double* sums, hipStream_t st);
hipError_t launch_icp_reduce_solve(const m3d_icp* s, hipStream_t st);
size_t eval_scratch_bytes(int64_t ns);
hipError_t launch_eval(const m3d_icp* s, int with_info, int32_t* idx, double* d2, double* partials,
                       double* out, hipStream_t st);
hipError_t launch_eval_fill(int64_t ns, int32_t* idx, double* d2, hipStream_t st);
hipError_t launch_cov_from_normals(const double* nrm, int64_t n, double eps, double* out, int width,
                                   hipStream_t st);
hipError_t launch_cov_pack(const double* cov9, const int32_t* slot, int64_t n, double* out6, hipStream_t st);
hipError_t launch_gicp_terms(const m3d_icp* s, double* cov_s, const double* cov_t, double* partials,
                             double* sums, bool with_defer, hipStream_t st);
hipError_t launch_robust_terms(const m3d_icp* s, int32_t kind, double k, double* cov_s, const double* cov_t,
                               double* partials, double* sums, bool with_defer, hipStream_t st);
hipError_t launch_color_gradients(const m3d_cloud* c, const double* nrm, const double* colors, const Grid* g,
                                  double radius, int k, double* rec, double* out3, hipStream_t st,
                                  const Grid* gf = nullptr, double hfine = 0.0);
hipError_t launch_color_rec_pack(const double* grad, const double* colors, int64_t n, double* rec, hipStream_t st);
hipError_t launch_intensity_pack(const double* colors, const int32_t* slot, int64_t n, double* out, hipStream_t st);
hipError_t launch_colored_terms(const m3d_icp* s, const double* rec_t, const double* is_s, double lambda,
                                int32_t kind, double k, double* partials, double* sums, bool with_defer,
                                hipStream_t st);
hipError_t launch_icp_terms_mode(const m3d_icp* s, int64_t off, const int32_t* claim,
                                 const int64_t* dmin, hipStream_t st);
hipError_t launch_icp_terms_reduce(const m3d_icp* s, int64_t off, const int32_t* claim,
                                   const int64_t* dmin, double* sums, bool reset_keys,
                                   hipStream_t st);
hipError_t launch_shard_winner(const m3d_icp* s, int64_t off, int64_t* dkey, hipStream_t st,
                               int64_t q0 = 0, int64_t q1 = -1);
hipError_t launch_shard_claim(const m3d_icp* s, const int64_t* dmin, int32_t* claim, hipStream_t st);
hipError_t launch_icp_solve(const m3d_icp* s, const double* sums, hipStream_t st);
hipError_t launch_icp_solve_state(IcpState* state, const double* sums, double relative_fitness, double relative_rmse,
                                  int32_t max_iteration, int32_t estimation, int64_t ns, const double* center,
                                  const FrameParams& f, hipStream_t st);
hipError_t grid_build(const float4* xyz32, int64_t n, double cell, hipStream_t st, Grid* g,
                      TmpArena* ta = nullptr, const float* lohi = nullptr);
hipError_t grid_occupancy(Grid* g, TmpArena* ta, hipStream_t st, unsigned long long* pin_dev = nullptr,
                          const unsigned long long* pin_host = nullptr);
void grid_free(Grid* g);
hipError_t launch_grid_nn(const float4* src32, int64_t ns, const Grid* qgrid, const Grid* g,
                          int64_t off, const IcpState* s, int64_t* keys, uint32_t* near2,
                          const int32_t* prev, const int64_t* dprev, const float4* tgt32, int64_t nt_shard,
                          hipStream_t st, int64_t q0 = 0, int64_t q1 = -1, int32_t* hlist = nullptr,
                          uint32_t* hcnt = nullptr, int32_t cand_cap = 0, const double* src64 = nullptr,
                          const double* tgt64 = nullptr, int32_t hcap = 0, int32_t xchunk = 0);
hipError_t morton_source(const m3d_cloud* src, double cell, m3d_cloud* out, Grid* gout, TmpArena* ta,
                         hipStream_t st);
hipError_t launch_corr_pairs(const int32_t* v, int64_t n, int32_t* cnt, int32_t* pairs, hipStream_t st);
hipError_t launch_scatter_i32(const int32_t* v, const int32_t* slot, int64_t n, int32_t* dst,
                              hipStream_t st);
hipError_t launch_scatter_f64(const double* v, const int32_t* slot, int64_t n, double* dst, hipStream_t st);
hipError_t launch_gather_i32(const int32_t* v, const int32_t* slot, int64_t n, int32_t* dst, hipStream_t st);
hipError_t launch_keys_to_idx(const int64_t* keys, int64_t n, int32_t* idx, hipStream_t st);
hipError_t launch_icp_set_T(const m3d_icp* s, const double* T_dev, hipStream_t st);
hipError_t launch_val_states(const m3d_icp* s, const double* T_dev, const int32_t* list, int64_t n,
                             IcpState* states, hipStream_t st);
int64_t validate_blocks(int64_t ns);
hipError_t launch_validate(const Grid* qgrid, int64_t ns, const double* src64, const Grid* g,
                           const double* tgt64, int64_t nt, const IcpState* states, int64_t nhyp,
                           double* part, double* out, hipStream_t st);
hipError_t build_mfma_tiles(const m3d_cloud* c, Grid* g, TmpArena* ta, hipStream_t st);
hipError_t grid_morton_perm(const Grid* g, TmpArena* ta, hipStream_t st, const int32_t** perm);

size_t voxel_scratch_bytes(int64_t n);
hipError_t voxel_down_sample(const double* xyz, const double* nrm, int64_t n, double voxel,
                             double* out_xyz, double* out_nrm, int64_t* out_n, void* scratch,
                             hipStream_t st, std::string* why);
double hybrid_fine_radius(const Grid* g, double radius, int k);
hipError_t hybrid_search(const m3d_cloud* c, const Grid* g, double radius, int k, int32_t* idx,
                         double* d2, int32_t* cnt, hipStream_t st, const Grid* gf = nullptr,
                         double hfine = 0.0);
// ... 88 lines not shown
```

### 3d-matching_amd/csrc/nn_brute.hip

```cpp
#include <algorithm>

#include "lds_dma.h"
#include "m3d_internal.h"
#include "nnkey.h"

#ifndef M3D_NN_BRUTE_PLAN_TU
#define M3D_NN_BRUTE_PLAN_TU 0
#endif
#ifndef M3D_NN_CLOCK
#define M3D_NN_CLOCK 0
#endif
#define M3D_NN_TU_MAIN (!M3D_NN_BRUTE_PLAN_TU)
#define M3D_NN_TU_PLAN_KERNEL (M3D_NN_BRUTE_PLAN_TU ? !M3D_NN_CLOCK : M3D_NN_CLOCK)
#if M3D_NN_TU_MAIN || M3D_NN_TU_PLAN_KERNEL

namespace m3d {

typedef _Float16 half8 __attribute__((ext_vector_type(8)));
typedef float floatx16 __attribute__((ext_vector_type(16)));

constexpr int kMG = 2;
constexpr int kMTile = 256;
constexpr int kTH = 4;
constexpr int kMTilePad = 1024;
constexpr int kMBlock = 512;
constexpr int kMQueries = (kMBlock / 64) * kMG * 32;

__device__ __forceinline__ void split16(float x, _Float16& hi, _Float16& lo) {
  hi = (_Float16)x;
  lo = (_Float16)(x - (float)hi);
}

union H8 {
  uint4 u;
  half8 h;
};

__device__ __forceinline__ uint32_t or16(const floatx16& k) {
  const auto b = [&](int i) { return __float_as_uint(k[i]); };
  const uint32_t o0 = __builtin_amdgcn_bitop3_b32(b(0), b(1), b(2), 0xFE);
  const uint32_t o1 = __builtin_amdgcn_bitop3_b32(b(3), b(4), b(5), 0xFE);
  const uint32_t o2 = __builtin_amdgcn_bitop3_b32(b(6), b(7), b(8), 0xFE);
  const uint32_t o3 = __builtin_amdgcn_bitop3_b32(b(9), b(10), b(11), 0xFE);
  const uint32_t o4 = __builtin_amdgcn_bitop3_b32(b(12), b(13), b(14), 0xFE);
  const uint32_t o5 = __builtin_amdgcn_bitop3_b32(o0, o1, o2, 0xFE);
  const uint32_t o6 = __builtin_amdgcn_bitop3_b32(o3, o4, b(15), 0xFE);
  return o5 | o6;
}

__device__ __forceinline__ void thr_operand(half8& b, float thr0, bool& force) {
  const float extra = 1.05f * ((32.0f * 1.01f * 5.9604645e-08f + 2.3841858e-07f) * fabsf(thr0) +
                               5.9604645e-08f);
  float thr = thr0 + extra;
  force = thr > 32768.0f;
  thr = fminf(fmaxf(thr, -32768.0f), 32768.0f);
  const _Float16 th = (_Float16)thr;
  const _Float16 tl = (_Float16)(thr - (float)th);
  b[3] = -th;
  b[4] = -tl;
}

#if M3D_NN_TU_MAIN
#ifndef M3D_NN_TILE_MORTON
#define M3D_NN_TILE_MORTON 1
#endif
__global__ __launch_bounds__(256) void pack16_sorted_kernel(const float4* __restrict__ sorted,
                                                            const int32_t* __restrict__ perm,
                                                            const float4* __restrict__ xyz32,
                                                            int64_t n, int64_t n_pad, float S,
                                                            uint4* __restrict__ mf16,
                                                            float4* __restrict__ mf32) {
  const int64_t k = (int64_t)blockIdx.x * 256 + threadIdx.x;
  if (k >= n_pad) return;
  H8 a, b;
  a.u = make_uint4(0, 0, 0, 0);
  b.u = make_uint4(0, 0, 0, 0);
  if (k < n) {
    const int32_t idx = __float_as_int(sorted[perm != nullptr ? perm[k] : k].w);
    const float4 t = xyz32[idx];
    _Float16 xh, xl, yh, yl, zh, zl, wh, wl;
    split16(t.x * S, xh, xl);
    split16(t.y * S, yh, yl);
    split16(t.z * S, zh, zl);
    split16(t.w * (S * S), wh, wl);
    a.h = half8{xh, xh, xl, yh, yh, yl, zh, zh};
    b.h = half8{zl, wh, wl, (_Float16)1, (_Float16)1, (_Float16)0, (_Float16)0, (_Float16)0};
    mf32[k] = make_float4(t.x, t.y, t.z, __int_as_float(idx));
  } else {
    b.h[1] = (_Float16)65504.0f;
    b.h[3] = (_Float16)1;
    b.h[4] = (_Float16)1;
    mf32[k] = make_float4(1.0e18f, 1.0e18f, 1.0e18f, __int_as_float(-1));
  }
  mf16[k] = a.u;
  mf16[n_pad + k] = b.u;
}

// ... 97 lines not shown
    xform32(Rt, p, qx, qy, qz);
    const int64_t key = sa.on == 0 ? keys[i]
                                   : seed_key_rec(s, sa.on == 2 ? sa.tgt[i] : seed_rec_prev(sa, i, off), qx, qy, qz);
    uint64_t k1 = key == kKeyNone ? make_key(r2_hi, 0xFFFFFFFFu) : (uint64_t)key;
    float k1d = key_real_d2(k1), n2 = kInf;
    const uint64_t k10 = k1;
    for (int64_t j = jb; j < je; ++j) {
      const float4 t = tgt32[j];
      if (__float_as_int(t.w) < 0) continue;
      const float d2 = d2f(qx, qy, qz, t.x, t.y, t.z);
      if (d2 <= r2_hi) near_push(k1, k1d, n2, make_key(d2, (uint32_t)(off + __float_as_int(t.w))), d2);
    }
    const bool pk = publish_k1(sa, bsy, k1, k1 != k10);
    if (pk || n2 < kInf) near_publish((unsigned long long*)&keys[i], &near2[i], k1, n2, pk);
  }
}

__device__ __forceinline__ void nn_push_rows(const float4 (&t)[16], int64_t off, float qx, float qy, float qz,
                                             float r2_hi, uint64_t& k1, float& k1d, float& n2) {
#pragma unroll
  for (int reg = 0; reg < 16; ++reg) {
    const float d2 = d2f(qx, qy, qz, t[reg].x, t[reg].y, t[reg].z);
    const uint64_t kc = make_key(d2, (uint32_t)(off + __float_as_int(t[reg].w)));
    if (d2 <= r2_hi) near_push(k1, k1d, n2, kc, d2);
  }
}

__device__ __forceinline__ void nn_exact_rows(const float4* __restrict__ rows, int64_t off, int h,
                                              float qx, float qy, float qz, float r2_hi,
                                              uint64_t& k1, float& k1d, float& n2) {
  float4 t[16];
#pragma unroll
  for (int reg = 0; reg < 16; ++reg) t[reg] = rows[(reg & 3) + 8 * (reg >> 2) + 4 * h];
  nn_push_rows(t, off, qx, qy, qz, r2_hi, k1, k1d, n2);
}

__device__ __forceinline__ uint64_t shfl_xor64(uint64_t v, int m) {
  const uint32_t lo = (uint32_t)__shfl_xor((int)(uint32_t)v, m);
  const uint32_t hi = (uint32_t)__shfl_xor((int)(uint32_t)(v >> 32), m);
  return ((uint64_t)hi << 32) | lo;
}

__device__ __forceinline__ uint32_t wave_or32(uint32_t v) {
  int x = (int)v;
  x |= __builtin_amdgcn_mov_dpp(x, 0xB1, 0xF, 0xF, false);
  x |= __builtin_amdgcn_mov_dpp(x, 0x4E, 0xF, 0xF, false);
  x |= xor4_dpp(x);
  x |= __builtin_amdgcn_mov_dpp(x, 0x128, 0xF, 0xF, false);
  return (uint32_t)(__builtin_amdgcn_readlane(x, 0) | __builtin_amdgcn_readlane(x, 16) |
                    __builtin_amdgcn_readlane(x, 32) | __builtin_amdgcn_readlane(x, 48));
}

template <bool kMax>
__device__ __forceinline__ float wave_minmax(float v) {
  const auto mm = [](float a, float b) { return kMax ? fmaxf(a, b) : fminf(a, b); };
  v = mm(v, __int_as_float(__builtin_amdgcn_mov_dpp(__float_as_int(v), 0xB1, 0xF, 0xF, false)));
  v = mm(v, __int_as_float(__builtin_amdgcn_mov_dpp(__float_as_int(v), 0x4E, 0xF, 0xF, false)));
  v = mm(v, __int_as_float(xor4_dpp(__float_as_int(v))));
  v = mm(v, __int_as_float(__builtin_amdgcn_mov_dpp(__float_as_int(v), 0x128, 0xF, 0xF, false)));
  const int x = __float_as_int(v);
  return mm(mm(__int_as_float(__builtin_amdgcn_readlane(x, 0)), __int_as_float(__builtin_amdgcn_readlane(x, 16))),
            mm(__int_as_float(__builtin_amdgcn_readlane(x, 32)), __int_as_float(__builtin_amdgcn_readlane(x, 48))));
}

#ifndef M3D_NN_CULL
#define M3D_NN_CULL 1
#endif
#ifndef M3D_NN_REACH
#define M3D_NN_REACH 1
#endif
#ifndef M3D_NN_ENTRY
#define M3D_NN_ENTRY 1
#endif
#ifndef M3D_NN_SEED_REC
#define M3D_NN_SEED_REC 1
#endif
#ifndef M3D_NN_DEFER_BATCH
#define M3D_NN_DEFER_BATCH 1
#endif
#ifndef M3D_NN_DEFER_FILTER
#define M3D_NN_DEFER_FILTER 1
#endif
#if M3D_NN_CLOCK
constexpr int kClkBlocks = 16384, kClkWords = 8;
__device__ unsigned long long g_nn_clock[kClkWords * kClkBlocks];
#endif
struct QBox {
  float lo[3], hi[3], X;
};
__device__ __forceinline__ bool box_out_of_reach(const QBox& q, const float4& tlo, const float4& thi) {
  const float gx = fmaxf(0.0f, fmaxf(q.lo[0] - thi.x, tlo.x - q.hi[0]));
  const float gy = fmaxf(0.0f, fmaxf(q.lo[1] - thi.y, tlo.y - q.hi[1]));
  const float gz = fmaxf(0.0f, fmaxf(q.lo[2] - thi.z, tlo.z - q.hi[2]));
  return d2f(gx, gy, gz, 0.0f, 0.0f, 0.0f) > q.X;
}
__device__ __forceinline__ bool point_out_of_reach(float qx, float qy, float qz, float X, const float (&lo)[3],
                                                   const float (&hi)[3]) {
  const float gx = fmaxf(0.0f, fmaxf(qx - hi[0], lo[0] - qx));
  const float gy = fmaxf(0.0f, fmaxf(qy - hi[1], lo[1] - qy));
  const float gz = fmaxf(0.0f, fmaxf(qz - hi[2], lo[2] - qz));
  return d2f(gx, gy, gz, 0.0f, 0.0f, 0.0f) > X;
}

constexpr int kTT = kTH * kMTile;
constexpr int kSub = kTT / 32;
constexpr uint64_t kGMask = (kSub == 64) ? ~0ull : ((1ull << kSub) - 1ull);
constexpr int kDefer = 16;
static_assert(kMBlock == 2 * kMTile, "one 16-B operand half per thread per half tile");
static_assert(kSub * kMG <= 64, "hit mask holds every (group, sub-tile)");
static_assert(kSub == 32, "one 32-bit hit record per group and tile");
static_assert(kMBlock / 64 == 8, "eight wave boxes, lanes ^1 ^2 ^4");

struct QState {
  float qx, qy, qz, qq;
  int64_t qi;
  uint64_t k1;
  float k1d, n2;
  half8 bq;
};

__device__ __forceinline__ uint64_t group_mask(uint32_t bits) {
  uint64_t m = 0;
#pragma unroll
  for (int g = 0; g < kMG; ++g)
    if ((bits >> g) & 1u) m |= kGMask << (g * kSub);
  return m;
}

__device__ __forceinline__ float load_query(QState& q, QBox& lq, int64_t slot, int h, float4 p, float4 rec,
                                            int64_t ns, const IcpState* __restrict__ s, const SeedArgs& sa,
                                            const int64_t* __restrict__ keys) {
  const float* Rt = s->Rt32;
  const float r2_hi = s->r2_hi, S = s->mfma_scale;
  const int64_t i = slot < ns ? slot : -1;
  q.qi = i;
  q.n2 = kInf;
  float X = -1.0f;
  if (i >= 0) {
    xform32(Rt, p, q.qx, q.qy, q.qz);
    const int64_t key = sa.on ? seed_key_rec(s, rec, q.qx, q.qy, q.qz) : keys[i];
    q.k1 = key == kKeyNone ? make_key(r2_hi, 0xFFFFFFFFu) : (uint64_t)key;
    X = search_bound(key_d2(q.k1), s->band_e, r2_hi);
    lq.lo[0] = fminf(lq.lo[0], q.qx);
    lq.lo[1] = fminf(lq.lo[1], q.qy);
    lq.lo[2] = fminf(lq.lo[2], q.qz);
    lq.hi[0] = fmaxf(lq.hi[0], q.qx);
    lq.hi[1] = fmaxf(lq.hi[1], q.qy);
    lq.hi[2] = fmaxf(lq.hi[2], q.qz);
    lq.X = fmaxf(lq.X, X);
  } else {
    q.qx = q.qy = q.qz = 0.0f;
    q.k1 = (uint64_t)kKeyNone;
  }
  q.k1d = key_real_d2(q.k1);
  q.qq = fmaf(q.qz, q.qz, fmaf(q.qy, q.qy, q.qx * q.qx));
  _Float16 ah, al, bh, bl, ch, cl;
  split16(-2.0f * S * q.qx, ah, al);
  split16(-2.0f * S * q.qy, bh, bl);
  split16(-2.0f * S * q.qz, ch, cl);
  const _Float16 one = (_Float16)1.0f, zero = (_Float16)0.0f;
  q.bq = h == 0 ? half8{ah, al, ah, bh, bl, bh, ch, cl} : half8{ch, one, one, zero, zero, zero, zero, zero};
  return X;
}

__device__ __forceinline__ bool refresh_threshold(QState& q, int h, float X, float eps, float S2) {
  bool fg;
  half8 bt = q.bq;
// ... 124 lines not shown
}

__device__ __forceinline__ void sweep_tile(uint32_t (&rec)[kMG], const uint4 (&t16)[2][2][kTT], int buf,
                                           int h, int c, uint32_t hmask, const QState (&q)[kMG],
                                           const floatx16& zacc) {
#pragma unroll
  for (int g = 0; g < kMG; ++g) rec[g] = 0;
  constexpr int kSteps = 8 * kMG;
#pragma unroll
  for (int half = 0; half < kTH; ++half) {
    if (!((hmask >> half) & 1u)) {
#pragma unroll
      for (int g = 0; g < kMG; ++g) rec[g] <<= 8;
      continue;
    }
    H8 av[8];
#pragma unroll
    for (int sub = 0; sub < 8; ++sub) av[sub].u = t16[buf][h][half * kMTile + sub * 32 + c];
    floatx16 kc = __builtin_amdgcn_mfma_f32_32x32x16_f16(av[0].h, q[0].bq, zacc, 0, 0, 0);
#pragma unroll
    for (int t = 0; t < kSteps; ++t) {
      floatx16 kn;
      if (t + 1 < kSteps)
        kn = __builtin_amdgcn_mfma_f32_32x32x16_f16(av[(t + 1) / kMG].h, q[(t + 1) % kMG].bq, zacc, 0, 0, 0);
      __builtin_amdgcn_sched_barrier(0);
      rec[t % kMG] = __builtin_amdgcn_alignbit(rec[t % kMG], or16(kc), 31);
      __builtin_amdgcn_sched_barrier(0);
      if (t + 1 < kSteps) kc = kn;
    }
  }
}

__device__ __forceinline__ uint64_t hit_mask(const uint32_t (&rec)[kMG], uint32_t hmask, uint64_t force64) {
  uint64_t hm = 0;
  uint32_t any = rec[0];
#pragma unroll
  for (int g = 1; g < kMG; ++g) any |= rec[g];
  if (__any(any != 0)) {
#pragma unroll
    for (int g = 0; g < kMG; ++g) hm |= (uint64_t)wave_or32(__builtin_bitreverse32(rec[g])) << (g * kSub);
  }
  uint32_t sm = 0;
#pragma unroll
  for (int half = 0; half < kTH; ++half)
    if ((hmask >> half) & 1u) sm |= 0xFFu << (8 * half);
  uint64_t fm = 0;
#pragma unroll
  for (int g = 0; g < kMG; ++g) fm |= (uint64_t)sm << (g * kSub);
  return hm | (force64 & fm);
}

__device__ __forceinline__ bool nn_exact_subtiles(uint64_t mg, const float4* __restrict__ tile, int64_t off,
                                                  int h, float r2_hi, QState& q) {
  const uint64_t kb = q.k1;
  while (mg != 0) {
    const int sub = __builtin_ctzll(mg);
    mg &= mg - 1;
    nn_exact_rows(tile + sub * 32, off, h, q.qx, q.qy, q.qz, r2_hi, q.k1, q.k1d, q.n2);
    const uint64_t o1 = shfl_xor64(q.k1, 32);
    const float on2 = __shfl_xor(q.n2, 32);
    near_merge(q.k1, q.k1d, q.n2, o1, on2);
  }
  return q.k1 != kb;
}

__device__ __forceinline__ uint32_t nn_defer_hits(const half8& a, const half8& bq, const floatx16& zacc) {
  const floatx16 v = __builtin_amdgcn_mfma_f32_32x32x16_f16(a, bq, zacc, 0, 0, 0);
  uint32_t m = 0;
#pragma unroll
  for (int reg = 15; reg >= 0; --reg) m = __builtin_amdgcn_alignbit(m, __float_as_uint(v[reg]), 31);
  return m;
}
__device__ __forceinline__ void nn_push_hits(uint32_t m, const float4* rows, int64_t off, int h, float qx,
                                             float qy, float qz, float r2_hi, uint64_t& k1, float& k1d,
                                             float& n2) {
  while (m != 0) {
    const int reg = __builtin_ctz(m);
    m &= m - 1;
    const float4 t = rows[(reg & 3) + 8 * (reg >> 2) + 4 * h];
    push_within(k1, k1d, n2, d2f(qx, qy, qz, t.x, t.y, t.z), r2_hi, (uint32_t)(off + __float_as_int(t.w)));
  }
}

template <bool kPlan>
__device__ __forceinline__ void nn_mfma_body(const float4* __restrict__ src32, int64_t ns,
                                             const uint4* __restrict__ tgt16, const float4* __restrict__ tgt32,
                                             const float4* __restrict__ tbox, int64_t nt_pad, int64_t off,
                                             const IcpState* __restrict__ s, int64_t* __restrict__ keys,
                                             uint32_t* __restrict__ near2, const SeedArgs& sa, int64_t q0,
                                             const NnPlan& pl) {
#if M3D_NN_ENTRY
  uint32_t e_tab = kPlanEmpty;
  if (kPlan && pl.table != nullptr) e_tab = pl.table[blockIdx.x];
  int32_t st_done = s->done, st_plan = s->plan_ok, st_mfma = s->mfma_ok;
  asm volatile("" : "+s"(st_done), "+s"(st_plan), "+s"(st_mfma), "+s"(e_tab));
  if (st_done) return;
#else
  if (s->done) return;
#endif
#if M3D_NN_CLOCK
  const unsigned long long clk0 = __builtin_amdgcn_s_memrealtime();
#endif
  NnSlice bs{0u, 0u, 0u};
  if (kPlan && pl.table != nullptr) {
#if M3D_NN_ENTRY
    if (st_plan) {
      const uint32_t e = e_tab;
#else
    if (s->plan_ok) {
      const uint32_t e = pl.table[blockIdx.x];
#endif
      if (e == kPlanEmpty) return;
      bs = NnSlice{plan_x(e), plan_y(e), plan_S(e)};
    } else {
      const unsigned y = blockIdx.x / (unsigned)pl.nq;
      if (y >= (unsigned)pl.S) return;
      bs = NnSlice{blockIdx.x - y * (unsigned)pl.nq, y, (unsigned)pl.S};
    }
  }
#if M3D_NN_ENTRY
  if (!st_mfma) {
#else
  if (!s->mfma_ok) {
#endif
    const int64_t tstep = (int64_t)(kPlan ? bs.S : gridDim.y) * kTT;
    for (int64_t t0 = (int64_t)(kPlan ? bs.y : blockIdx.y) * kTT; t0 < nt_pad; t0 += tstep)
      nn_slice_scan(src32, ns, tgt32, t0, min(nt_pad, t0 + kTT), off, s, keys, near2, sa, q0,
                    kPlan ? bs.x : blockIdx.x, kPlan ? bs.y : blockIdx.y);
    return;
  }
  __shared__ uint4 t16[2][2][kTT];
  __shared__ uint64_t dlist[kMBlock / 64][kDefer];
  __shared__ uint32_t dtile[kMBlock / 64][kDefer];
  __shared__ float4 qbox[kMBlock / 64][2];
  __shared__ uint64_t rslot[2][kMBlock / 64];
#if M3D_NN_CLOCK
  __shared__ uint32_t clk_slow, clk_ticket;
  __shared__ unsigned long long clk_exit;
  if (threadIdx.x == 0) {
    clk_slow = 0;
    clk_ticket = 0;
    clk_exit = 0;
  }
  uint32_t clk_halves = 0;
#endif
  uint32_t kept = 0;
  __shared__ uint32_t slice_xy;
  if (kPlan && threadIdx.x == 0) slice_xy = bs.x | (bs.y << 16);
  const int lane = threadIdx.x & 63, wave = threadIdx.x >> 6;
  const int c = lane & 31, h = lane >> 5;
  const float r2_hi = s->r2_hi, eps = s->screen_eps_m, S = s->mfma_scale, be = s->band_e;
  const float S2 = S * S;

  QState q[kMG];
  uint32_t act = 0;
  uint32_t force = 0;
  uint32_t chg = 0;
  QBox lq{{kInf, kInf, kInf}, {-kInf, -kInf, -kInf}, -1.0f};
  const int64_t slot0 = q0 + (kPlan ? (int64_t)bs.x : (int64_t)blockIdx.x) * kMQueries + wave * kMG * 32 + c;
  float4 qp[kMG], qr[kMG];
#pragma unroll
  for (int g = 0; g < kMG; ++g) {
    const int64_t slot = slot0 + g * 32;
    qp[g] = src32[slot < ns ? slot : 0];
    qr[g] = make_float4(0.0f, 0.0f, 0.0f, 0.0f);
  }
  if (sa.on == 2) {
#pragma unroll
    for (int g = 0; g < kMG; ++g) {
      const int64_t slot = slot0 + g * 32;
      qr[g] = sa.tgt[slot < ns ? slot : 0];
    }
  } else if (sa.on) {
#pragma unroll
    for (int g = 0; g < kMG; ++g) {
      const int64_t slot = slot0 + g * 32;
      qr[g] = seed_rec_prev(sa, slot < ns ? slot : 0, off);
    }
  }
#pragma unroll
  for (int g = 0; g < kMG; ++g) {
    const int64_t slot = slot0 + g * 32;
    const float X = load_query(q[g], lq, slot, h, qp[g], qr[g], ns, s, sa, keys);
    if (q[g].qi >= 0) act |= 1u << g;
    if (__any(refresh_threshold(q[g], h, X, eps, S2))) force |= 1u << g;
  }
  const floatx16 zacc = {0.0f, 0.0f, 0.0f, 0.0f, 0.0f, 0.0f, 0.0f, 0.0f,
                         0.0f, 0.0f, 0.0f, 0.0f, 0.0f, 0.0f, 0.0f, 0.0f};
  uint32_t dfr = 0;
#pragma unroll
  for (int g = 0; g < kMG; ++g)
    if (!((force >> g) & 1u) && __all(q[g].qi < 0 || key_real(q[g].k1))) dfr |= 1u << g;
  int dn = 0;
  uint64_t dmask = group_mask(dfr);
  dmask = ((uint64_t)(uint32_t)__builtin_amdgcn_readfirstlane((int)(dmask >> 32)) << 32) |
          (uint32_t)__builtin_amdgcn_readfirstlane((int)(uint32_t)dmask);

  const QBox bx = reduce_boxes(lq, qbox, lane, wave);
  const int ntile = (int)(nt_pad / kTT);
  const ReachArgs ra{q, act, be, r2_hi, rslot, wave};
  TileCursor cur{tbox, qbox[wave], bx, lane, ntile, (int)(kPlan ? bs.S : gridDim.y), (int)(kPlan ? bs.y : blockIdx.y), 0, 0};
  cur.cull_round(ra);
  int t0, t1;
  uint32_t h0, h1;
  cur.next(t0, h0, ra);
  if (t0 < ntile) stage_tile(t16[0], tgt16, nt_pad, t0, false);
  const uint64_t force64 = group_mask(force);
  __syncthreads();
#if M3D_NN_CLOCK
  const unsigned long long clk1 = __builtin_amdgcn_s_memrealtime();
#endif
  int tog = 0;
  for (; t0 < ntile; t0 = t1, h0 = h1) {
    const int buf = kPlan ? (int)(kept & 1u) : tog;
    const int64_t j0 = (int64_t)t0 * kTT;
    if (kPlan || M3D_NN_CLOCK) ++kept;
#if M3D_NN_CLOCK
    clk_halves += (uint32_t)__builtin_popcount(h0);
#endif
    cur.next(t1, h1, ra);
    if (t1 < ntile) stage_tile(t16[buf ^ 1], tgt16, nt_pad, t1, true);
    uint32_t rec[kMG];
    sweep_tile(rec, t16, buf, h, c, h0, q, zacc);
    uint64_t hm = hit_mask(rec, h0, force64);
    const uint64_t hd = hm & dmask;
    if (hd != 0 && dn < kDefer) {
      if (lane == 0) {
        dlist[wave][dn] = hd;
        dtile[wave][dn] = (uint32_t)j0;
      }
      ++dn;
// ... 53 lines not shown
#pragma unroll
      for (int g = 0; g < kMG; ++g) gs |= (uint32_t)((ent >> (g * kSub + sub)) & 1u) << g;
    };
    uint64_t kb[kMG];
#pragma unroll
    for (int g = 0; g < kMG; ++g) kb[g] = q[g].k1;
    for (;;) {
      uint32_t gsel = 0;
      float4 ld[kStash / 2];
#if M3D_NN_DEFER_FILTER
      H8 av[kStash];
#endif
#pragma unroll
      for (int k = 0; k < kStash / 2; ++k) {
        uint32_t ra, ga, rb, gb;
        pop(ra, ga);
        pop(rb, gb);
        gsel |= (ga | (gb << kMG)) << (2 * kMG * k);
        ld[k] = make_float4(0.0f, 0.0f, 0.0f, 0.0f);
        if (h == 0 ? ga != 0 : gb != 0) ld[k] = tgt32[(int64_t)(h == 0 ? ra : rb) + c];
#if M3D_NN_DEFER_FILTER
        av[2 * k].u = tgt16[(int64_t)h * nt_pad + ra + c];
        av[2 * k + 1].u = tgt16[(int64_t)h * nt_pad + rb + c];
#endif
      }
#pragma unroll
      for (int k = 0; k < kStash / 2; ++k) stash[(2 * k + h) * 32 + c] = ld[k];
      __builtin_amdgcn_fence(__ATOMIC_RELEASE, "wavefront");
      __builtin_amdgcn_wave_barrier();
      __builtin_amdgcn_fence(__ATOMIC_ACQUIRE, "wavefront");
#if M3D_NN_DEFER_FILTER
#pragma unroll
      for (int sl = 0; sl < kStash; ++sl) {
        const uint32_t gs = (gsel >> (kMG * sl)) & ((1u << kMG) - 1u);
        if (gs == 0) break;
        uint32_t hit[kMG];
#pragma unroll
        for (int g = 0; g < kMG; ++g) hit[g] = (gs >> g) & 1u ? nn_defer_hits(av[sl].h, q[g].bq, zacc) : 0u;
#pragma unroll
        for (int g = 0; g < kMG; ++g)
          if ((gs >> g) & 1u)
            nn_push_hits(hit[g], stash + sl * 32, off, h, q[g].qx, q[g].qy, q[g].qz, r2_hi, q[g].k1, q[g].k1d,
                         q[g].n2);
      }
#else
#pragma unroll 1
      for (int sl = 0; sl < kStash; ++sl) {
        const uint32_t gs = (gsel >> (kMG * sl)) & ((1u << kMG) - 1u);
        if (gs == 0) break;
        float4 t[16];
#pragma unroll
        for (int reg = 0; reg < 16; ++reg) t[reg] = stash[sl * 32 + (reg & 3) + 8 * (reg >> 2) + 4 * h];
#pragma unroll
        for (int g = 0; g < kMG; ++g)
          if ((gs >> g) & 1u) nn_push_rows(t, off, q[g].qx, q[g].qy, q[g].qz, r2_hi, q[g].k1, q[g].k1d, q[g].n2);
      }
#endif
      if (U == 0 && e + 1 >= dn) break;
      __builtin_amdgcn_fence(__ATOMIC_RELEASE, "wavefront");
      __builtin_amdgcn_wave_barrier();
    }
#pragma unroll
    for (int g = 0; g < kMG; ++g) {
      const uint64_t o1 = shfl_xor64(q[g].k1, 32);
      const float on2 = __shfl_xor(q[g].n2, 32);
      near_merge(q[g].k1, q[g].k1d, q[g].n2, o1, on2);
      chg |= (uint32_t)(q[g].k1 != kb[g]) << g;
    }
  }
#else
  for (int e = 0; e < dn; ++e) {
    const uint64_t ent = dlist[wave][e];
    const float4* tile = tgt32 + (int64_t)dtile[wave][e];
#pragma unroll
    for (int g = 0; g < kMG; ++g)
      chg |= (uint32_t)nn_exact_subtiles((ent >> (g * kSub)) & kGMask, tile, off, h, r2_hi, q[g]) << g;
  }
#endif
#if M3D_NN_CLOCK
  const unsigned long long clk2b = __builtin_amdgcn_s_memrealtime();
#endif
  const uint32_t sxy = kPlan ? slice_xy : 0u;
  const int64_t sxl = (int64_t)(sxy & 0xFFFFu);
  const unsigned syl = sxy >> 16;
#define M3D_NN_SX (kPlan ? sxl : (int64_t)blockIdx.x)
#define M3D_NN_SY (kPlan ? syl : blockIdx.y)
#pragma unroll
  for (int g = 0; g < kMG; ++g) {
    if (h != 0 || q[g].qi < 0) continue;
#if (M3D_NN_CULL && M3D_NN_REACH) || M3D_NN_DEFER_BATCH
    int cq = c;
    asm volatile("" : "+v"(cq));
    const int64_t qi = q0 + M3D_NN_SX * kMQueries + (wave * kMG + g) * 32 + cq;
#else
    const int64_t qi = q[g].qi;
#endif
    const bool pk = publish_k1(sa, M3D_NN_SY, q[g].k1, (chg >> g) & 1u);
    if (pk || q[g].n2 < kInf) near_publish((unsigned long long*)&keys[qi], &near2[qi], q[g].k1, q[g].n2, pk);
  }
  if (kPlan && pl.cnt != nullptr && threadIdx.x == 0) atomicAdd(&pl.cnt[M3D_NN_SX], kept);
#if M3D_NN_CLOCK
  {
    const unsigned long long clk3 = __builtin_amdgcn_s_memrealtime();
    const int64_t blk = (int64_t)blockIdx.y * gridDim.x + blockIdx.x;
    if (lane == 0) {
      atomicMax(&clk_exit, clk3);
      if (atomicAdd(&clk_ticket, 1u) == kMBlock / 64 - 1 && blk < kClkBlocks) {
        unsigned long long* rec = g_nn_clock + kClkWords * blk;
        rec[0] = clk0;
        rec[1] = clk1;
        rec[2] = clk2;
        rec[3] = atomicMax(&clk_exit, 0ull);
        rec[4] = kept;
        rec[5] = atomicMax(&clk_slow, 0u);
        rec[6] = (unsigned long long)M3D_NN_SX | ((unsigned long long)M3D_NN_SY << 32) | ((unsigned long long)cur.ty << 48);
        rec[7] = clk2b;
      }
    }
  }
#endif
}

#undef M3D_NN_SX
#undef M3D_NN_SY
#define M3D_NN_KERNEL_ARGS                                                                            \
  const float4 *__restrict__ src32, int64_t ns, const uint4 *__restrict__ tgt16,                      \
      const float4 *__restrict__ tgt32, const float4 *__restrict__ tbox, int64_t nt_pad, int64_t off, \
      const IcpState *__restrict__ s, int64_t *__restrict__ keys, uint32_t *__restrict__ near2, SeedArgs sa, int64_t q0
#if M3D_NN_TU_MAIN
__global__ __launch_bounds__(kMBlock) __attribute__((amdgpu_waves_per_eu(4))) void nn_mfma_kernel(M3D_NN_KERNEL_ARGS) {
  nn_mfma_body<false>(src32, ns, tgt16, tgt32, tbox, nt_pad, off, s, keys, near2, sa, q0, NnPlan{nullptr, nullptr, 0, 0});
}
#endif
hipError_t launch_nn_plan_kernel(unsigned blocks, hipStream_t st, M3D_NN_KERNEL_ARGS, NnPlan pl);
int nn_plan_kernel_blocks_per_cu();
#if M3D_NN_TU_PLAN_KERNEL
__global__ __launch_bounds__(kMBlock) __attribute__((amdgpu_waves_per_eu(4))) void nn_mfma_plan_kernel(
    M3D_NN_KERNEL_ARGS, NnPlan pl) {
  nn_mfma_body<true>(src32, ns, tgt16, tgt32, tbox, nt_pad, off, s, keys, near2, sa, q0, pl);
}
hipError_t launch_nn_plan_kernel(unsigned blocks, hipStream_t st, M3D_NN_KERNEL_ARGS, NnPlan pl) {
  nn_mfma_plan_kernel<<<dim3(blocks), kMBlock, 0, st>>>(src32, ns, tgt16, tgt32, tbox, nt_pad, off, s, keys, near2, sa,
                                                        q0, pl);
  return hipGetLastError();
}
int nn_plan_kernel_blocks_per_cu() {
  int per = 0;
  if (hipOccupancyMaxActiveBlocksPerMultiprocessor(&per, nn_mfma_plan_kernel, kMBlock, 0) != hipSuccess) return 0;
  return per > 0 ? per : 1;
}
#endif
#undef M3D_NN_KERNEL_ARGS
#if M3D_NN_TU_MAIN

static int64_t nn_grid_y(int64_t bx, int64_t ntiles, int64_t slots, bool cull) {
  const auto clamped = [&](int64_t S) { return std::min(std::max<int64_t>(S, 1), ntiles); };
  const int64_t s0 = clamped((2048 + bx - 1) / bx);
  if (slots <= 0 || ntiles <= 1) {
    const int64_t per = (ntiles + s0 - 1) / s0;
    return (ntiles + per - 1) / per;
  }
  if (cull) return clamped(slots / bx);
  int64_t best = s0;
  double best_eff = 0.0;
  for (int64_t S = s0; S <= std::min(2 * s0, ntiles); ++S) {
    const int64_t blocks = bx * S, rounds = (blocks + slots - 1) / slots;
    const double eff = (double)blocks / (double)(rounds * slots);
    if (eff > best_eff + 1e-9) {
      best_eff = eff;
      best = S;
    }
  }
  return best;
}

#if M3D_NN_CLOCK
}
extern "C" int m3d_debug_nn_clock(unsigned long long* out, int n) {
  return hipMemcpyFromSymbol(out, HIP_SYMBOL(m3d::g_nn_clock), sizeof(unsigned long long) * (size_t)n) == hipSuccess ? 0 : -1;
}
namespace m3d {
#endif
static bool icp_nn_uses_mfma(const m3d_icp* s) {
  return s->tgrid != nullptr && s->tgrid->mf16 != nullptr;
}

bool icp_nn_range_ok(const m3d_icp* s) {
  if (s->params.nn_method == M3D_NN_GRID) return s->sgrid != nullptr && s->sgrid->mpts != nullptr;
  return icp_nn_uses_mfma(s);
}

hipError_t launch_icp_nn(const m3d_icp* s, int64_t off, bool self_seed, hipStream_t st, int64_t q0,
                         int64_t q1) {
  const int64_t ns = q1 < 0 ? s->src->n : q1;
  if (ns <= q0 || s->tgt->n == 0) return hipSuccess;
  const Grid* tg = s->tgrid;
  const int64_t tt = (int64_t)kTH * kMTile;
  if (!icp_nn_uses_mfma(s) || tg->mf_npad % tt != 0) return hipErrorInvalidValue;
  const int64_t slots = nn_resident_slots();
  const int64_t bx = (ns - q0 + kMQueries - 1) / kMQueries;
  const int64_t gy = nn_grid_y(bx, tg->mf_npad / tt, slots, M3D_NN_CULL != 0);
  const bool by_rec = M3D_NN_SEED_REC != 0 && self_seed && off == 0 && s->tgt->rec64 != nullptr && s->seed != nullptr;
  const SeedArgs sa{s->corr, by_rec ? s->seed : s->tgt->xyz32, s->tgt->n, by_rec ? 2 : self_seed ? 1 : 0};
  const bool planned = nn_plan_on() && s->nn_qblocks > 0 && q0 == 0 && ns == s->src->n && bx == s->nn_qblocks &&
                       bx * gy <= s->nn_budget;
  if (planned)
    return launch_nn_plan_kernel((unsigned)s->nn_budget, st, s->src->xyz32, ns, tg->mf16, tg->mf32, tg->mfbox,
                                 tg->mf_npad, off, s->state, s->keys, s->near2, sa, q0,
                                 NnPlan{s->nn_table, s->nn_cnt, (int)bx, (int)gy});
  nn_mfma_kernel<<<dim3((unsigned)bx, (unsigned)gy), kMBlock, 0, st>>>(
        s->src->xyz32, ns, tg->mf16, tg->mf32, tg->mfbox, tg->mf_npad, off, s->state, s->keys, s->near2, sa, q0);
  return hipGetLastError();
}

int64_t nn_resident_slots() {
  static const int64_t slots = [] {
    int dev = 0, per = 0;
    hipDeviceProp_t p;
    if (hipGetDevice(&dev) != hipSuccess || hipGetDeviceProperties(&p, dev) != hipSuccess) return (int64_t)0;
    if (hipOccupancyMaxActiveBlocksPerMultiprocessor(&per, nn_mfma_kernel, kMBlock, 0) != hipSuccess)
      return (int64_t)0;
    const int pp = nn_plan_kernel_blocks_per_cu();
    per = per > 0 ? per : 1;
    if (pp > 0 && pp < per) per = pp;
    return (int64_t)p.multiProcessorCount * per;
  }();
  return slots;
}

bool nn_plan_on() {
  static const bool on = [] {
    const char* e = getenv("M3D_NN_PLAN");
    return !(e && atoi(e) == 0);
  }();
  return on;
}

void nn_plan_shape(int64_t ns, int32_t* qblocks, int32_t* budget) {
  const int64_t slots = nn_resident_slots(), bx = (ns + kMQueries - 1) / kMQueries;
  const bool ok = M3D_NN_CULL != 0 && slots > 0 && bx >= 1 && bx < slots && bx <= kPlanMaxQ && slots <= 0xFFFF;
  *qblocks = ok ? (int32_t)bx : 0;
  *budget = ok ? (int32_t)slots : 0;
}

PlanArgs nn_plan_args(const m3d_icp* s) {
  PlanArgs pa;
  if (!nn_plan_on() || s->nn_qblocks <= 0 || s->tgrid == nullptr) return pa;
  pa.cnt = s->nn_cnt;
  pa.seen = s->nn_seen;
  pa.table = s->nn_table;
  pa.n = s->nn_qblocks;
  pa.budget = s->nn_budget;
  pa.cap = (int32_t)plan_cap(kPlanSmax, s->tgrid->mf_npad / ((int64_t)kTH * kMTile));
  return pa;
}

#endif

}
#endif
```

### 3d-matching_amd/m3d/_lib.py

```python

from __future__ import annotations

import ctypes as C
import os
from pathlib import Path

LIB_PATH = Path(__file__).resolve().parent / "libm3d.so"

M3D_OK = 0
M3D_ERR_INVALID = -1
M3D_ERR_HIP = -2
M3D_ERR_OOM = -3
M3D_ERR_NODEVICE = -4
M3D_ERR_COMM = -5

HYP_OK, HYP_DEGENERATE, HYP_NONFINITE = 0, 1, 2
SCORE_SQUARED, SCORE_NORM = 0, 1
EST_POINT_TO_POINT, EST_POINT_TO_PLANE = 0, 1
KERNEL_NN, KERNEL_SCORE, KERNEL_KABSCH, KERNEL_TERMS, KERNEL_LOOP, KERNEL_COMM = 0, 1, 2, 3, 4, 5
ICP_NO_SPLIT = 2
NN_BRUTE, NN_GRID = 0, 1
EVAL_INFORMATION = 1
ROBUST_L2, ROBUST_L1, ROBUST_HUBER, ROBUST_CAUCHY, ROBUST_GM, ROBUST_TUKEY = 0, 1, 2, 3, 4, 5
COMM_ID_BYTES = 128
# ... 148 lines not shown
                                        C.POINTER(dbl), vp, vp]),
    "m3d_gicp_run_robust": (C.c_int, [vp, vp, vp, vp, vp, C.POINTER(dbl), dbl, C.POINTER(GicpParams),
                                      C.POINTER(RobustKernel), C.POINTER(IcpResult), vp, vp]),
    "m3d_color_gradients": (C.c_int, [vp, vp, vp, dbl, i32, vp, vp]),
    "m3d_colored_terms": (C.c_int, [vp, vp, vp, vp, vp, vp, C.POINTER(dbl), dbl, i32, dbl, C.POINTER(RobustKernel),
                                    C.POINTER(dbl), vp, vp]),
    "m3d_colored_icp_run": (C.c_int, [vp, vp, vp, vp, vp, vp, C.POINTER(dbl), dbl, C.POINTER(ColoredParams),
                                      C.POINTER(RobustKernel), C.POINTER(IcpResult), vp, vp]),
    "m3d_icp_run": (C.c_int, [vp, vp, vp, C.POINTER(dbl), dbl, C.POINTER(IcpParams),
                              C.POINTER(IcpResult), vp, vp]),
    "m3d_icp_create": (C.c_int, [vp, vp, vp, dbl, C.POINTER(IcpParams), C.POINTER(vp)]),
    "m3d_icp_destroy": (None, [vp]),
    "m3d_icp_reset": (C.c_int, [vp, C.POINTER(dbl), vp]),
    "m3d_icp_step": (C.c_int, [vp, vp]),
    "m3d_icp_steps": (C.c_int, [vp, C.c_int32, vp]),
    "m3d_icp_prepare_steps": (C.c_int, [vp, C.c_int32]),
    "m3d_icp_shard_nn": (C.c_int, [vp, i64, vp, vp]),
    "m3d_icp_shard_nn_range": (C.c_int, [vp, i64, i64, i64, vp, vp]),
    "m3d_icp_shard_claim": (C.c_int, [vp, vp, vp, vp]),
    "m3d_icp_shard_terms": (C.c_int, [vp, i64, vp, vp, vp, vp]),
    "m3d_icp_solve": (C.c_int, [vp, vp, vp]),
    "m3d_icp_result_get": (C.c_int, [vp, C.POINTER(IcpResult), vp]),
    "m3d_icp_set_source_total": (C.c_int, [vp, i64]),
    "m3d_icp_corr": (vp, [vp]),
    "m3d_icp_copy_corr": (C.c_int, [vp, vp, vp]),
    "m3d_corr_pairs": (C.c_int, [vp, vp, i64, vp, C.POINTER(i64), vp]),
    "m3d_icp_copy_slots": (C.c_int, [vp, vp, vp]),
    "m3d_icp_copy_points": (C.c_int, [vp, vp, vp]),
    "m3d_voxel_down_sample": (C.c_int, [vp, vp, vp, i64, dbl, vp, vp, C.POINTER(i64), vp]),
    "m3d_hybrid_search": (C.c_int, [vp, vp, dbl, i32, vp, vp, vp, vp]),
    "m3d_estimate_normals": (C.c_int, [vp, vp, dbl, i32, vp, vp]),
    "m3d_compute_fpfh": (C.c_int, [vp, vp, vp, dbl, i32, vp, vp]),
    "m3d_knn_search": (C.c_int, [vp, vp, i32, vp, vp, vp, vp]),
    "m3d_estimate_normals_knn": (C.c_int, [vp, vp, i32, vp, vp]),
    "m3d_remove_statistical_outlier": (C.c_int, [vp, vp, i32, dbl, vp, C.POINTER(i64),
                                                 C.POINTER(OutlierStats), vp, vp]),
    "m3d_remove_radius_outlier": (C.c_int, [vp, vp, i32, dbl, vp, C.POINTER(i64), vp, vp]),
    "m3d_segment_plane": (C.c_int, [vp, vp, C.POINTER(PlaneParams), vp, C.POINTER(PlaneResult), vp, vp, vp, vp]),
    "m3d_plane_score": (C.c_int, [vp, vp, vp, i64, dbl, vp, vp, vp]),
    "m3d_plane_chunk": (i32, []),
    "m3d_cluster_dbscan": (C.c_int, [vp, vp, dbl, i32, vp, C.POINTER(DbscanResult), vp, vp, vp]),
    "m3d_model_resolution": (C.c_int, [vp, vp, C.POINTER(dbl), vp]),
    "m3d_compute_iss_keypoints": (C.c_int, [vp, vp, C.POINTER(IssParams), C.POINTER(IssResult), vp, vp, vp, vp]),
    "m3d_feature_correspondences": (C.c_int, [vp, vp, i64, vp, i64, i32, i32, dbl, vp,
                                              C.POINTER(i64), vp]),
    "m3d_ransac_on_correspondences": (C.c_int, [vp, vp, vp, vp, i64, C.POINTER(FeatureRansacParams),
                                                C.POINTER(FeatureRansacResult), vp, vp]),
    "m3d_fgr_on_correspondences": (C.c_int, [vp, vp, vp, vp, i64, C.POINTER(FgrParams), C.POINTER(FgrResult),
                                             vp, vp, vp]),
    "m3d_fgr_tuple_test": (C.c_int, [vp, vp, vp, vp, i64, C.POINTER(FgrParams), vp, C.POINTER(i64),
                                     C.POINTER(i64), vp]),
    "m3d_fgr_terms": (C.c_int, [vp, vp, vp, i64, dbl, C.POINTER(dbl), vp]),
    "m3d_fgr_trial_batch": (i32, []),
    "m3d_fgr_one_wg_rows": (i32, []),
    "m3d_mesh_create": (C.c_int, [vp, vp, i64, vp, i64, C.POINTER(vp)]),
    "m3d_mesh_destroy": (None, [vp]),
    "m3d_mesh_size": (i64, [vp]),
    "m3d_mesh_closest": (C.c_int, [vp, vp, vp, i64, C.POINTER(dbl), i32, dbl, vp, vp, vp, vp, vp, vp]),
    "m3d_mesh_icp_terms": (C.c_int, [vp, vp, vp, C.POINTER(dbl), dbl, C.POINTER(RobustKernel), i32, vp,
                                     C.POINTER(dbl), vp, vp, vp]),
    "m3d_mesh_icp_run": (C.c_int, [vp, vp, vp, C.POINTER(dbl), dbl, C.POINTER(IcpParams), C.POINTER(RobustKernel),
                                   i32, i32, C.POINTER(IcpResult), vp, vp]),
    "m3d_mesh_grid_info": (C.c_int, [vp, C.POINTER(i64)]),
    "m3d_mesh_brute_tile": (i32, []),
    "m3d_mesh_auto_brute_max": (i32, []),
    "m3d_comm_unique_id": (C.c_int, [C.POINTER(C.c_uint8)]),
    "m3d_comm_init": (C.c_int, [vp, C.POINTER(C.c_uint8), C.c_int, C.c_int, C.POINTER(vp)]),
    "m3d_comm_destroy": (None, [vp]),
    "m3d_comm_allreduce": (C.c_int, [vp, vp, i64, C.c_int, C.c_int, vp]),
    "m3d_icp_shard_steps": (C.c_int, [vp, vp, i64, i32, vp]),
    "m3d_icp_source_shard_steps": (C.c_int, [vp, vp, i32, vp]),
    "m3d_ransac_best_allreduce": (C.c_int, [vp, vp, i64, vp, vp]),
    "m3d_ransac_run_sharded": (C.c_int, [vp, vp, vp, C.POINTER(RansacParams), C.POINTER(RansacResult), vp]),
    "m3d_comm_poisoned": (C.c_int, [vp]),
    "m3d_debug_comm_inject": (C.c_int, [vp, C.c_int]),
    "m3d_debug_acos_cr": (C.c_int, [vp, C.c_int64, vp]),
    "m3d_debug_acos_device": (C.c_int, [vp, vp, C.c_int64, vp, C.c_int, vp]),
    "m3d_debug_block_cache_fill": (C.c_int, [C.c_int]),
    "m3d_debug_icp_defer_count": (C.c_int, [vp, C.c_uint32, vp]),
    "m3d_debug_nn_plan_host": (C.c_int, [vp, C.c_int64, C.c_int64, C.c_int64, C.c_int64, vp]),
    "m3d_debug_icp_nn_plan": (C.c_int, [vp, vp, C.c_int64, vp]),
    "m3d_debug_icp_nn_plan_read": (C.c_int, [vp, vp, vp, vp, vp]),
    "m3d_debug_icp_seed_read": (C.c_int, [vp, vp, vp, vp, vp, vp]),
    "m3d_parse_ascii_rows": (C.c_int, [C.c_char_p, C.c_size_t, i64, i32, C.POINTER(dbl),
                                       C.POINTER(C.c_size_t)]),
    "m3d_format_ascii_rows": (C.c_int, [C.POINTER(dbl), i64, i32, vp, C.c_size_t, C.POINTER(C.c_size_t)]),
    "m3d_merge_vertices": (C.c_int, [C.POINTER(dbl), i64, C.POINTER(dbl), C.POINTER(i32), C.POINTER(i64)]),
    "m3d_content_keys": (C.c_int, [C.POINTER(vp), C.POINTER(C.c_size_t), i32, C.POINTER(u64)]),
    "m3d_debug_xxh64": (u64, [vp, C.c_size_t, u64]),
    "m3d_debug_xxh3_128": (C.c_int, [vp, C.c_size_t, C.POINTER(u64)]),
    "m3d_debug_kabsch3_host":(C.c_int, [C.POINTER(dbl), C.POINTER(dbl), C.POINTER(dbl)]),
    "m3d_debug_ldlt6_host": (C.c_int, [C.POINTER(dbl), C.POINTER(dbl), C.POINTER(dbl)]),
    "m3d_debug_sym3_eigenvalues_host": (C.c_int, [C.POINTER(dbl), C.POINTER(dbl)]),
    "m3d_debug_sym3_eigen_host": (C.c_int, [C.POINTER(dbl), C.POINTER(dbl), C.POINTER(dbl)]),
}

_lib = None


class M3DError(RuntimeError):
    pass


class M3DCommError(M3DError):
    """A peer rank failed, or the communicator was aborted after a failure (M3D_ERR_COMM)."""


def load() -> C.CDLL:
    global _lib
    if _lib is not None:
        return _lib
    if not LIB_PATH.exists():
        raise ImportError(f"{LIB_PATH} not built: run `make -C {LIB_PATH.parent.parent / 'csrc'}` "
                          "(hipcc --offload-arch=gfx950)")
    try:
        import torch
    except ImportError:
        pass
    lib = C.CDLL(os.fspath(LIB_PATH))
    lib.m3d_abi_version.restype = C.c_int
    if lib.m3d_abi_version() != ABI_VERSION:
        raise ImportError(f"{LIB_PATH}: ABI {lib.m3d_abi_version()} != {ABI_VERSION}; rebuild it")
    for name, (res, args) in SIGNATURES.items():
        f = getattr(lib, name, None)
        if f is None and name.startswith("m3d_debug_") and os.environ.get("AB_LIB"):
            continue
        if f is None:
            raise ImportError(f"{LIB_PATH}: no symbol {name}; rebuild it")
        f.restype = res
        f.argtypes = args
    _lib = lib
    return lib


def check(rc: int, ctx=None, what: str = "") -> None:
    if rc == M3D_OK:
        return
    msg = ""
    if ctx is not None:
        raw = load().m3d_last_error(ctx)
        msg = raw.decode() if raw else ""
    if rc == M3D_ERR_INVALID:
        raise ValueError(f"{what}: {msg}" if msg else what)
    if rc == M3D_ERR_COMM:
        raise M3DCommError(f"{what} failed (code {rc}): {msg}")
    raise M3DError(f"{what} failed (code {rc}): {msg}")
```

### include/m3d.h

```cpp
#ifndef M3D_H_
#define M3D_H_

#include <stddef.h>
#include <stdint.h>

#ifdef __cplusplus
extern "C" {
#endif

#define M3D_ABI_VERSION 13

#define M3D_OK 0
#define M3D_ERR_INVALID (-1)
#define M3D_ERR_HIP (-2)
#define M3D_ERR_OOM (-3)
#define M3D_ERR_NODEVICE (-4)
#define M3D_ERR_COMM (-5)

#define M3D_HYP_OK 0
#define M3D_HYP_DEGENERATE 1
#define M3D_HYP_NONFINITE 2

#define M3D_SCORE_SQUARED 0
#define M3D_SCORE_NORM 1
// ... 336 lines not shown
} m3d_feature_ransac_params;

typedef struct {
  double T[16];
  double fitness;
  double inlier_rmse;
  int64_t best_index;
  int64_t validations;
  double corres_ratio;
} m3d_feature_ransac_result;

int m3d_ransac_on_correspondences(m3d_ctx* ctx, const m3d_cloud* src, const m3d_cloud* tgt,
                                  const int32_t* corr, int64_t nc,
                                  const m3d_feature_ransac_params* params,
                                  m3d_feature_ransac_result* out, int32_t* corr_set_out,
                                  void* stream);

typedef struct {
  double division_factor;
  double maximum_correspondence_distance;
  double tuple_scale;
  uint64_t seed;
  int32_t iteration_number;
  int32_t maximum_tuple_count;
  int32_t use_absolute_scale;
  int32_t decrease_mu;
  int32_t tuple_test;
  int32_t path;
} m3d_fgr_params;
typedef struct {
  double T[16];
  double fitness, inlier_rmse;
  int64_t n_input, n_rows;
  int64_t tuples, trials;
  double par_final, scale_global;
  double mean_src[3], mean_tgt[3];
  double T_norm[16];
} m3d_fgr_result;
int m3d_fgr_on_correspondences(m3d_ctx* ctx, const m3d_cloud* src, const m3d_cloud* tgt, const int32_t* corr,
                               int64_t nc, const m3d_fgr_params* params, m3d_fgr_result* out,
                               int32_t* rows_out, int32_t* corr_set_out, void* stream);
int m3d_fgr_tuple_test(m3d_ctx* ctx, const m3d_cloud* src, const m3d_cloud* tgt, const int32_t* corr,
                       int64_t nc, const m3d_fgr_params* params, int32_t* rows_out, int64_t* n_rows_out,
                       int64_t* trials_out, void* stream);
int m3d_fgr_terms(m3d_ctx* ctx, const double* p, const double* q, int64_t n, double par, double* sums27_out,
                  void* stream);
int32_t m3d_fgr_trial_batch(void);
int32_t m3d_fgr_one_wg_rows(void);

int m3d_mesh_create(m3d_ctx* ctx, const double* vertices, int64_t nv, const int32_t* triangles, int64_t nf,
                    m3d_mesh** out);
void m3d_mesh_destroy(m3d_mesh* mesh);
int64_t m3d_mesh_size(const m3d_mesh* mesh);
int m3d_mesh_closest(m3d_ctx* ctx, m3d_mesh* mesh, const double* xyz, int64_t n, const double* T, int32_t path,
                     double r0, double* d2_out, int32_t* tri_out, double* point_out, double* uv_out,
                     uint8_t* region_out, void* stream);
int m3d_mesh_grid_info(const m3d_mesh* mesh, int64_t* out4);
int32_t m3d_mesh_brute_tile(void);
int32_t m3d_mesh_auto_brute_max(void);

int m3d_mesh_icp_terms(m3d_ctx* ctx, m3d_mesh* mesh, const m3d_cloud* src, const double* T_host, double max_dist,
                       const m3d_robust_kernel* kernel, int32_t path, const int32_t* seed_tri, double* sums_out,
                       int32_t* tri_idx, double* d2_out, void* stream);
int m3d_mesh_icp_run(m3d_ctx* ctx, m3d_mesh* mesh, const m3d_cloud* src, const double* init, double max_dist,
                     const m3d_icp_params* params, const m3d_robust_kernel* kernel, int32_t path, int32_t seed,
                     m3d_icp_result* out, int32_t* tri_idx, void* stream);

int m3d_debug_kabsch3_host(const double* src9, const double* tgt9, double* T16);
int m3d_debug_ldlt6_host(const double* A36, const double* b6, double* x6);
int m3d_debug_sym3_eigenvalues_host(const double* sym6, double* lam3);
int m3d_debug_sym3_eigen_host(const double* sym6, double* lam3, double* V9);
uint64_t m3d_debug_xxh64(const void* p, size_t len, uint64_t seed);
int m3d_debug_xxh3_128(const void* p, size_t len, uint64_t* out2);
int m3d_debug_comm_inject(m3d_comm* c, int what);
int m3d_debug_acos_cr(const double* u, int64_t n, double* out);
int m3d_debug_acos_device(m3d_ctx* ctx, const double* u, int64_t n, double* out, int mode, void* stream);
int m3d_debug_block_cache_fill(int byte);
int m3d_debug_icp_defer_count(m3d_icp* s, uint32_t count, void* stream);
int m3d_debug_nn_plan_host(const uint32_t* counts, int64_t n, int64_t budget, int64_t smax, int64_t ntiles,
                           uint32_t* out);
int m3d_debug_icp_nn_plan(m3d_icp* s, const int32_t* S, int64_t n, void* stream);
int m3d_debug_icp_nn_plan_read(m3d_icp* s, uint32_t* counts, uint32_t* table, int32_t* shape3, void* stream);
int m3d_debug_icp_seed_read(m3d_icp* s, float* seed, int32_t* corr, float* tgt32, int32_t* info2, void* stream);


int m3d_parse_ascii_rows(const char* buf, size_t len, int64_t rows, int32_t cols, double* out,
                         size_t* consumed);
int m3d_format_ascii_rows(const double* data, int64_t rows, int32_t cols, char* out, size_t cap,
                          size_t* written);
int m3d_merge_vertices(const double* xyz, int64_t n, double* uniq, int32_t* inverse,
                       int64_t* n_unique);
int m3d_content_keys(const void* const* bufs, const size_t* lens, int32_t n, uint64_t* keys);

#ifdef __cplusplus
}
#endif
#endif
```

Before: 20550 ICP iter/s (100k src x 100k tgt per GPU).

## Fuse ICP terms computation into planned brute-force NN kernel via per-query-block tickets

Adds an NN kernel variant that, once all target slices of a query block have finished (tracked by per-block ticket counters), computes that block's point-to-plane terms partials inline. A single-block reduce+solve kernel then follows, replacing the separate terms/solve pass. This is meant to remove a full kernel launch and the re-read of keys/near2 from a separate pass, and to overlap terms work with the NN scan tail. In exchange it adds atomics, extra counters, a device-side args struct set up at creation, and an occupancy cap that may lower resident slots for the plain NN kernels too.

```diff
diff --git a/3d-matching_amd/csrc/api.cpp b/3d-matching_amd/csrc/api.cpp
--- a/3d-matching_amd/csrc/api.cpp
+++ b/3d-matching_amd/csrc/api.cpp
@@ -1186,7 +1186,7 @@
 }
 
 hipError_t enqueue_nn(m3d_icp* s, int64_t off, hipStream_t st, bool self_seed = false, int64_t q0 = 0,
-                      int64_t q1 = -1) {
+                      int64_t q1 = -1, bool with_terms = false) {
   m3d_ctx* ctx = s->ctx;
   const bool whole = q0 == 0 && (q1 < 0 || q1 == s->src->n);
   const bool seeded = self_seed && s->keys_clean && off == 0 && whole;
@@ -1202,7 +1202,7 @@
     if (e != hipSuccess) return e;
   }
   KTimer kt(ctx, M3D_KERNEL_NN, st);
-  return launch_icp_nn(s, off, seeded, st, q0, q1);
+  return launch_icp_nn(s, off, seeded, st, q0, q1, with_terms);
 }
 }
 
@@ -1297,7 +1297,8 @@
       cv.add(&s->state, 1);
       if (params->nn_method == M3D_NN_BRUTE) nn_plan_shape(src->n, &s->nn_qblocks, &s->nn_budget);
       if (s->nn_qblocks > 0) {
-        cv.add(&s->nn_cnt, (size_t)s->nn_qblocks);
+        cv.add(&s->nn_cnt, 2 * (size_t)s->nn_qblocks);
+        cv.add(&s->nn_targs, (nn_terms_dev_bytes() + 7) / 8);
         cv.add(&s->nn_seen, (size_t)s->nn_qblocks);
         cv.add(&s->nn_table, (size_t)s->nn_budget);
       }
@@ -1324,8 +1325,17 @@
         hipMemsetAsync(s->hcnt, 0, kDeferWords * sizeof(uint32_t), nullptr) != hipSuccess)
       grc = m3d_fail(ctx, M3D_ERR_HIP, "loop arrays: deferral counter");
     if (!grc && s->nn_cnt != nullptr &&
-        hipMemsetAsync(s->nn_cnt, 0, (size_t)s->nn_qblocks * sizeof(uint32_t), nullptr) != hipSuccess)
+        hipMemsetAsync(s->nn_cnt, 0, 2 * (size_t)s->nn_qblocks * sizeof(uint32_t), nullptr) != hipSuccess)
       grc = m3d_fail(ctx, M3D_ERR_HIP, "loop arrays: NN plan counters");
+    if (!grc && s->nn_cnt != nullptr) {
+      s->nn_tix = s->nn_cnt + s->nn_qblocks;
+      s->src = src_m;
+      s->tgt = tgt;
+      s->tgrid = tg;
+      s->params = *params;
+      if (launch_nn_terms_setup(s, nullptr) != hipSuccess)
+        grc = m3d_fail(ctx, M3D_ERR_HIP, "loop arrays: NN terms arguments");
+    }
     if (!grc) {
       hipError_t e = hipStreamSynchronize(nullptr);
       if (e != hipSuccess) grc = m3d_fail(ctx, M3D_ERR_HIP, std::string("loop setup: ") + hipGetErrorString(e));
@@ -1424,6 +1434,28 @@
   }();
   return env && (keys_back || s->nblocks <= 256);
 }
+
+bool nn_terms_env() {
+  static const bool on = [] {
+    const char* e = getenv("M3D_NN_TERMS");
+    return !(e && atoi(e) == 0);
+  }();
+  return on;
+}
+
+NnTermsSel nn_terms_sel(const m3d_icp* s, bool fused, bool reset) {
+  NnTermsSel c;
+  c.planned = s->params.nn_method == M3D_NN_BRUTE && s->nn_targs != nullptr && icp_nn_planned(s);
+  c.fused = fused;
+  c.reset = reset;
+  c.p2plane = s->params.estimation == M3D_EST_POINT_TO_PLANE;
+  c.rec64 = s->tgt->rec64 != nullptr;
+  c.seed = s->seed != nullptr;
+  c.claim = false;
+  c.one_device = s->ns_total == 0;
+  c.on = nn_terms_env() && !s->nn_terms_off;
+  return c;
+}
 }
 
 int m3d_icp_step(m3d_icp* s, void* stream) {
@@ -1433,6 +1465,13 @@
   hipStream_t st = S(stream);
   const bool reset = s->params.nn_method != M3D_NN_GRID && s->src->n > 0;
   const bool fused = fused_tail(s, reset);
+  if (nn_terms_selected(nn_terms_sel(s, fused, reset))) {
+    HIPX(ctx, enqueue_nn(s, 0, st, true, 0, -1, true));
+    KTimer kt(ctx, M3D_KERNEL_TERMS, st);
+    HIPX(ctx, launch_icp_reduce_solve_block(s, st));
+    s->keys_clean = true;
+    return M3D_OK;
+  }
   HIPX(ctx, enqueue_nn(s, 0, st, fused));
   if (fused) {
     KTimer kt(ctx, M3D_KERNEL_TERMS, st);
@@ -3207,4 +3246,41 @@
   return M3D_OK;
 }
 
-}
+int m3d_debug_icp_nn_terms(m3d_icp* s, int on) {
+  if (!s) return M3D_ERR_INVALID;
+  s->nn_terms_off = on == 0;
+  for (int k = 0; k < 2; ++k) {
+    if (s->graph[k] != nullptr) hipGraphExecDestroy(s->graph[k]);
+    s->graph[k] = nullptr;
+    s->graph_n[k] = s->seen_n[k] = -1;
+  }
+  const bool reset = s->params.nn_method != M3D_NN_GRID && s->src->n > 0;
+  return nn_terms_selected(nn_terms_sel(s, fused_tail(s, reset), reset)) ? 1 : 0;
+}
+
+int m3d_debug_icp_nn_terms_read(m3d_icp* s, uint32_t* tickets, uint32_t* counts, void* stream) {
+  if (!s) return M3D_ERR_INVALID;
+  if (s->nn_tix == nullptr) return 0;
+  Touch tch{s->ctx, S(stream)};
+  const size_t bytes = sizeof(uint32_t) * (size_t)s->nn_qblocks;
+  if (tickets) HIPX(s->ctx, hipMemcpyAsync(tickets, s->nn_tix, bytes, hipMemcpyDeviceToHost, S(stream)));
+  if (counts) HIPX(s->ctx, hipMemcpyAsync(counts, s->nn_cnt, bytes, hipMemcpyDeviceToHost, S(stream)));
+  HIPX(s->ctx, hipStreamSynchronize(S(stream)));
+  return s->nn_qblocks;
+}
+
+int m3d_debug_nn_terms_select(uint32_t bits) {
+  NnTermsSel c;
+  c.planned = bits & 1u;
+  c.fused = bits & 2u;
+  c.reset = bits & 4u;
+  c.p2plane = bits & 8u;
+  c.rec64 = bits & 16u;
+  c.seed = bits & 32u;
+  c.claim = bits & 64u;
+  c.one_device = bits & 128u;
+  c.on = bits & 256u;
+  return nn_terms_selected(c) ? 1 : 0;
+}
+
+}
diff --git a/3d-matching_amd/csrc/icp.hip b/3d-matching_amd/csrc/icp.hip
--- a/3d-matching_amd/csrc/icp.hip
+++ b/3d-matching_amd/csrc/icp.hip
@@ -17,6 +17,10 @@
 constexpr double kU = 5.9604644775390625e-08;
 constexpr double kU64 = 1.1102230246251565e-16;
 
+#ifndef M3D_ICP_TERMS_ONLY
+#define M3D_ICP_TERMS_ONLY 0
+#endif
+#if !M3D_ICP_TERMS_ONLY
 
 __device__ __forceinline__ float f32_ru(double d) {
   const float f = (float)d;
@@ -151,6 +155,7 @@
   near2[i] = kNearNone;
 }
 
+#endif
 template <bool k32>
 __device__ __forceinline__ double swap_add(double a, double b) {
   const uint64_t ua = (uint64_t)__double_as_longlong(a), ub = (uint64_t)__double_as_longlong(b);
@@ -240,6 +245,11 @@
   int64_t* reset_keys;
   float4* seed;
 };
+struct NnTermsDev {
+  TermsArgs a;
+  double* partials;
+  uint32_t* tix;
+};
 
 #if M3D_TAIL_CLOCK
 __device__ unsigned long long g_tail_clock[3 * 4096 + 24];
@@ -256,9 +266,9 @@
   do {             \
   } while (0)
 #endif
-template <bool kWT, int kEst>
+template <bool kWT, int kEst, bool kSc1 = false>
 __device__ __forceinline__ void terms_block(const TermsArgs& a, const IcpState* __restrict__ s,
-                                            double* __restrict__ partials) {
+                                            double* __restrict__ partials, const unsigned bx) {
   __shared__ double red[kTermSlots][kTermsBlock / kWave];
 #if M3D_TERMS_CLOCK
   unsigned long long tph_[8];
@@ -278,13 +288,18 @@
   float n2[kP];
 #pragma unroll
   for (int u = 0; u < kP; ++u) {
-    const int64_t i = ((int64_t)blockIdx.x * kP + u) * kTermsBlock + threadIdx.x;
+    const int64_t i = ((int64_t)bx * kP + u) * kTermsBlock + threadIdx.x;
     valid[u] = i < a.ns;
     ii[u] = valid[u] ? i : 0;
     gj[u] = -1;
     d2[u] = 0.0;
     fixed[u] = true;
-    if (a.claim == nullptr) {
+    if (kSc1) {
+      k1[u] = valid[u] ? (uint64_t)__hip_atomic_load(&a.keys[ii[u]], __ATOMIC_RELAXED, __HIP_MEMORY_SCOPE_AGENT)
+                       : (uint64_t)kKeyNone;
+      n2[u] = valid[u] ? __uint_as_float(__hip_atomic_load(&a.near2[ii[u]], __ATOMIC_RELAXED, __HIP_MEMORY_SCOPE_AGENT))
+                       : kInf;
+    } else if (a.claim == nullptr) {
       k1[u] = valid[u] ? (uint64_t)a.keys[ii[u]] : (uint64_t)kKeyNone;
       n2[u] = valid[u] ? __uint_as_float(a.near2[ii[u]]) : kInf;
     } else if (valid[u]) {
@@ -316,7 +331,7 @@
       amb[u] = X[u] >= 0.0f && n2[u] <= X[u];
 #if M3D_TAIL_CLOCK
       {
-        const int64_t gw = (int64_t)blockIdx.x * (kTermsBlock / kWave) + threadIdx.x / kWave;
+        const int64_t gw = (int64_t)bx * (kTermsBlock / kWave) + threadIdx.x / kWave;
         const int na = __popcll(__ballot(amb[u]));
         if ((threadIdx.x & (kWave - 1)) == 0 && gw < 4096) g_tail_clock[2 * 4096 + 8 + gw] = na;
       }
@@ -407,7 +422,7 @@
     double v = 0.0;
     if (threadIdx.x < 30)
       for (int w = 0; w < kTermsBlock / kWave; ++w) v += red[threadIdx.x][w];
-    double* dst = partials + (int64_t)blockIdx.x * kTermSlots + threadIdx.x;
+    double* dst = partials + (int64_t)bx * kTermSlots + threadIdx.x;
     if (kWT)
       __hip_atomic_store(reinterpret_cast<unsigned long long*>(dst), __double_as_longlong(v),
                          __ATOMIC_RELAXED, __HIP_MEMORY_SCOPE_AGENT);
@@ -417,18 +432,19 @@
   M3D_TPH(7);
 #if M3D_TERMS_CLOCK
   {
-    const int64_t gw = (int64_t)blockIdx.x * (kTermsBlock / kWave) + threadIdx.x / kWave;
+    const int64_t gw = (int64_t)bx * (kTermsBlock / kWave) + threadIdx.x / kWave;
     if ((threadIdx.x & (kWave - 1)) == 0 && gw < 4096)
       for (int k = 0; k < 8; ++k) g_terms_clock[8 * gw + k] = tph_[k];
   }
 #endif
 }
 
+#if !M3D_ICP_TERMS_ONLY
 template <int kEst>
 __global__ __launch_bounds__(kTermsBlock) void terms_kernel(TermsArgs a, const IcpState* __restrict__ s,
                                                             double* __restrict__ partials) {
   if (s->done) return;
-  terms_block<false, kEst>(a, s, partials);
+  terms_block<false, kEst>(a, s, partials, blockIdx.x);
 }
 
 __global__ __launch_bounds__(256) void shard_winner_kernel(
@@ -758,6 +774,65 @@
 struct PlanNone {
   static constexpr int32_t n = 0;
 };
+template <int kEst, bool kPlanner, class Plan>
+__device__ __forceinline__ void reduce_solve_block(IcpState* s, double* partials, int64_t nblocks,
+                                                   double* __restrict__ sums, const SolveParams& sp, int do_solve,
+                                                   const Plan& pa) {
+  __shared__ double red[kReduceGroups][kTermSlots];
+  M3D_TCLK(0);
+  SolveIn in;
+  if (do_solve && threadIdx.x < kWave) solve_in(s, in);
+  const bool planner = kPlanner && pa.n > 0 && threadIdx.x >= kWave && threadIdx.x < 2 * kWave;
+  PlanIn pin;
+  if constexpr (kPlanner)
+    if (planner) plan_in(pa, s, threadIdx.x - kWave, pin);
+  const int slot = threadIdx.x & (kTermSlots - 1);
+  constexpr int kG = kReduceGroups / (kTermsBlock / kTermSlots);
+  double gv[kG];
+#pragma unroll
+  for (int u = 0; u < kG; ++u) gv[u] = 0.0;
+  const int g0 = threadIdx.x / kTermSlots;
+  constexpr int kR = 8;
+  for (int64_t b0 = 0; b0 < nblocks; b0 += kR * kReduceGroups) {
+    double t[kR][kG];
+#pragma unroll
+    for (int r = 0; r < kR; ++r)
+#pragma unroll
+      for (int u = 0; u < kG; ++u) {
+        const int64_t b = b0 + r * kReduceGroups + g0 + u * (kTermsBlock / kTermSlots);
+        t[r][u] = b < nblocks
+                      ? __longlong_as_double(__hip_atomic_load(
+                            reinterpret_cast<unsigned long long*>(partials + b * kTermSlots + slot),
+                            __ATOMIC_RELAXED, __HIP_MEMORY_SCOPE_AGENT))
+                      : 0.0;
+      }
+#pragma unroll
+    for (int r = 0; r < kR; ++r)
+#pragma unroll
+      for (int u = 0; u < kG; ++u) gv[u] += t[r][u];
+  }
+  M3D_TCLK(8);
+#pragma unroll
+  for (int u = 0; u < kG; ++u) red[g0 + u * (kTermsBlock / kTermSlots)][slot] = gv[u];
+  __syncthreads();
+  if (threadIdx.x < kTermSlots) {
+    double t = 0.0;
+    for (int k = 0; k < kReduceGroups; ++k) t += red[k][threadIdx.x];
+    red[0][threadIdx.x] = t;
+    sums[threadIdx.x] = t;
+  }
+  M3D_TCLK(9);
+  __syncthreads();
+  M3D_TCLK(1);
+  if (threadIdx.x < kWave) {
+    if (threadIdx.x == 0) s->ticket = 0;
+    if (do_solve) solve_state<kEst>(red[0], s, sp, in);
+  } else if (planner) {
+    if constexpr (kPlanner) plan_wave(pa, s, threadIdx.x - kWave, pin);
+  }
+  M3D_TCLK(2);
+}
+
 template <int kEst, bool kPlanner>
 __global__ __launch_bounds__(kTermsBlock) void terms_solve_kernel(
     TermsArgs a, IcpState* s, double* partials, int64_t nblocks, double* __restrict__ sums,
@@ -766,7 +841,7 @@
 #if M3D_TAIL_CLOCK
   const unsigned long long clk0 = __builtin_amdgcn_s_memrealtime();
 #endif
-  terms_block<true, kEst>(a, s, partials);
+  terms_block<true, kEst>(a, s, partials, blockIdx.x);
 #if M3D_TAIL_CLOCK
   {
     const unsigned long long clk1 = __builtin_amdgcn_s_memrealtime();
@@ -840,6 +915,13 @@
     if constexpr (kPlanner) plan_wave(pa, s, threadIdx.x - kWave, pin);
   }
   M3D_TCLK(2);
+}
+
+__global__ __launch_bounds__(kTermsBlock) void reduce_solve_kernel(IcpState* s, double* partials, int64_t nblocks,
+                                                                   double* __restrict__ sums, SolveParams sp,
+                                                                   PlanArgs pa) {
+  if (s->done) return;
+  reduce_solve_block<M3D_EST_POINT_TO_PLANE, true>(s, partials, nblocks, sums, sp, 1, pa);
 }
 
 __global__ __launch_bounds__(256) void nn_finalize_kernel(const double* __restrict__ pcd64,
@@ -995,7 +1077,7 @@
 
 static hipError_t reset_plan_counts(const m3d_icp* s, hipStream_t st) {
   if (s->nn_cnt == nullptr) return hipSuccess;
-  return hipMemsetAsync(s->nn_cnt, 0, (size_t)s->nn_qblocks * sizeof(uint32_t), st);
+  return hipMemsetAsync(s->nn_cnt, 0, (size_t)s->nn_qblocks * sizeof(uint32_t) * (s->nn_tix != nullptr ? 2 : 1), st);
 }
 
 hipError_t launch_icp_state_init(IcpState* state, const double* T, bool apply_init, double r2, const FrameParams& f,
@@ -1252,6 +1334,25 @@
   return hipGetLastError();
 }
 
+__global__ void store_nn_terms_kernel(NnTermsDev v, NnTermsDev* dst) { *dst = v; }
+
+size_t nn_terms_dev_bytes() { return sizeof(NnTermsDev); }
+
+hipError_t launch_nn_terms_setup(const m3d_icp* s, hipStream_t st) {
+  NnTermsDev v;
+  v.a = terms_args(s, 0, nullptr, nullptr, true);
+  v.partials = s->partials;
+  v.tix = s->nn_tix;
+  store_nn_terms_kernel<<<1, 1, 0, st>>>(v, reinterpret_cast<NnTermsDev*>(s->nn_targs));
+  return hipGetLastError();
+}
+
+hipError_t launch_icp_reduce_solve_block(const m3d_icp* s, hipStream_t st) {
+  reduce_solve_kernel<<<1, kTermsBlock, 0, st>>>(s->state, s->partials, s->nblocks, s->sums, solve_params(s),
+                                                 nn_plan_args(s));
+  return hipGetLastError();
+}
+
 hipError_t launch_nn_finalize(const m3d_icp* s, int32_t* idx, double* d2, hipStream_t st) {
   const int64_t ns = s->src->n;
   if (ns == 0) return hipSuccess;
@@ -1315,6 +1416,7 @@
 
 int64_t terms_blocks(int64_t ns) { return ns > 0 ? (ns + kTermsBlock - 1) / kTermsBlock : 1; }
 
+#endif
 }
 
 #if M3D_TERMS_CLOCK
diff --git a/3d-matching_amd/csrc/m3d_internal.h b/3d-matching_amd/csrc/m3d_internal.h
--- a/3d-matching_amd/csrc/m3d_internal.h
+++ b/3d-matching_amd/csrc/m3d_internal.h
@@ -337,6 +337,9 @@
   uint32_t* nn_table = nullptr;
   int32_t nn_qblocks = 0;
   int32_t nn_budget = 0;
+  uint32_t* nn_tix = nullptr;
+  uint64_t* nn_targs = nullptr;
+  bool nn_terms_off = false;
   int32_t* corr = nullptr;
   float4* seed = nullptr;
   double* pcd64 = nullptr;
@@ -439,7 +442,25 @@
 hipError_t launch_icp_keyinit(const m3d_icp* s, int64_t shard_offset, hipStream_t st, int64_t q0 = 0,
                               int64_t q1 = -1);
 hipError_t launch_icp_nn(const m3d_icp* s, int64_t shard_offset, bool self_seed, hipStream_t st,
-                         int64_t q0 = 0, int64_t q1 = -1);
+                         int64_t q0 = 0, int64_t q1 = -1, bool with_terms = false);
+struct NnTermsSel {
+  bool planned;
+  bool fused;
+  bool reset;
+  bool p2plane;
+  bool rec64;
+  bool seed;
+  bool claim;
+  bool one_device;
+  bool on;
+};
+inline bool nn_terms_selected(const NnTermsSel& c) {
+  return c.planned && c.fused && c.reset && c.p2plane && c.rec64 && c.seed && !c.claim && c.one_device && c.on;
+}
+bool icp_nn_planned(const m3d_icp* s);
+size_t nn_terms_dev_bytes();
+hipError_t launch_nn_terms_setup(const m3d_icp* s, hipStream_t st);
+hipError_t launch_icp_reduce_solve_block(const m3d_icp* s, hipStream_t st);
 int64_t nn_resident_slots();
 bool nn_plan_on();
 void nn_plan_shape(int64_t ns, int32_t* qblocks, int32_t* budget);
diff --git a/3d-matching_amd/csrc/nn_brute.hip b/3d-matching_amd/csrc/nn_brute.hip
--- a/3d-matching_amd/csrc/nn_brute.hip
+++ b/3d-matching_amd/csrc/nn_brute.hip
@@ -10,9 +10,21 @@
 #ifndef M3D_NN_CLOCK
 #define M3D_NN_CLOCK 0
 #endif
-#define M3D_NN_TU_MAIN (!M3D_NN_BRUTE_PLAN_TU)
-#define M3D_NN_TU_PLAN_KERNEL (M3D_NN_BRUTE_PLAN_TU ? !M3D_NN_CLOCK : M3D_NN_CLOCK)
-#if M3D_NN_TU_MAIN || M3D_NN_TU_PLAN_KERNEL
+#ifndef M3D_NN_BRUTE_TERMS_TU
+#define M3D_NN_BRUTE_TERMS_TU 0
+#endif
+#define M3D_NN_TU_MAIN (!M3D_NN_BRUTE_PLAN_TU && !M3D_NN_BRUTE_TERMS_TU)
+#define M3D_NN_TU_PLAN_KERNEL (M3D_NN_BRUTE_PLAN_TU ? !M3D_NN_CLOCK : (M3D_NN_TU_MAIN && M3D_NN_CLOCK))
+#define M3D_NN_TU_TERMS_KERNEL (M3D_NN_BRUTE_TERMS_TU ? !M3D_NN_CLOCK : (M3D_NN_TU_MAIN && M3D_NN_CLOCK))
+#if M3D_NN_TU_MAIN || M3D_NN_TU_PLAN_KERNEL || M3D_NN_TU_TERMS_KERNEL
+#if M3D_NN_TU_TERMS_KERNEL
+#undef M3D_TAIL_CLOCK
+#undef M3D_TERMS_CLOCK
+#define M3D_TAIL_CLOCK 0
+#define M3D_TERMS_CLOCK 0
+#define M3D_ICP_TERMS_ONLY 1
+#include "icp.hip"
+#endif
 
 namespace m3d {
 
@@ -276,7 +288,7 @@
 #define M3D_NN_DEFER_FILTER 1
 #endif
 #if M3D_NN_CLOCK
-constexpr int kClkBlocks = 16384, kClkWords = 8;
+constexpr int kClkBlocks = 16384, kClkWords = 10;
 __device__ unsigned long long g_nn_clock[kClkWords * kClkBlocks];
 #endif
 struct QBox {
@@ -567,13 +579,39 @@
   }
 }
 
-template <bool kPlan>
+#if M3D_NN_TU_TERMS_KERNEL
+__device__ __forceinline__ void nn_terms_handoff(const NnTermsDev* __restrict__ td, const IcpState* __restrict__ s,
+                                                 unsigned x, unsigned S, unsigned long long* clk = nullptr) {
+  __shared__ uint32_t tk_last;
+  asm volatile("s_waitcnt vmcnt(0)" ::: "memory");
+  __syncthreads();
+  if (threadIdx.x == 0) {
+    const uint32_t t = __hip_atomic_fetch_add(&td->tix[x], 1u, __ATOMIC_RELAXED, __HIP_MEMORY_SCOPE_AGENT);
+    tk_last = t == S - 1u ? 1u : 0u;
+#if M3D_NN_CLOCK
+    if (clk != nullptr) {
+      clk[8] = __builtin_amdgcn_s_memrealtime();
+      clk[9] = 0;
+    }
+#endif
+  }
+  __syncthreads();
+  if (!tk_last) return;
+  terms_block<true, M3D_EST_POINT_TO_PLANE, true>(td->a, s, td->partials, x);
+  if (threadIdx.x == 0) __hip_atomic_store(&td->tix[x], 0u, __ATOMIC_RELAXED, __HIP_MEMORY_SCOPE_AGENT);
+#if M3D_NN_CLOCK
+  if (clk != nullptr && threadIdx.x == 0) clk[9] = __builtin_amdgcn_s_memrealtime();
+#endif
+}
+#endif
+
+template <bool kPlan, bool kTerms = false>
 __device__ __forceinline__ void nn_mfma_body(const float4* __restrict__ src32, int64_t ns,
                                              const uint4* __restrict__ tgt16, const float4* __restrict__ tgt32,
                                              const float4* __restrict__ tbox, int64_t nt_pad, int64_t off,
                                              const IcpState* __restrict__ s, int64_t* __restrict__ keys,
                                              uint32_t* __restrict__ near2, const SeedArgs& sa, int64_t q0,
-                                             const NnPlan& pl) {
+                                             const NnPlan& pl, const void* td = nullptr) {
 #if M3D_NN_ENTRY
   uint32_t e_tab = kPlanEmpty;
   if (kPlan && pl.table != nullptr) e_tab = pl.table[blockIdx.x];
@@ -612,6 +650,9 @@
     for (int64_t t0 = (int64_t)(kPlan ? bs.y : blockIdx.y) * kTT; t0 < nt_pad; t0 += tstep)
       nn_slice_scan(src32, ns, tgt32, t0, min(nt_pad, t0 + kTT), off, s, keys, near2, sa, q0,
                     kPlan ? bs.x : blockIdx.x, kPlan ? bs.y : blockIdx.y);
+#if M3D_NN_TU_TERMS_KERNEL
+    if constexpr (kTerms) nn_terms_handoff(static_cast<const NnTermsDev*>(td), s, bs.x, bs.S);
+#endif
     return;
   }
   __shared__ uint4 t16[2][2][kTT];
@@ -631,7 +672,7 @@
 #endif
   uint32_t kept = 0;
   __shared__ uint32_t slice_xy;
-  if (kPlan && threadIdx.x == 0) slice_xy = bs.x | (bs.y << 16);
+  if (kPlan && threadIdx.x == 0) slice_xy = bs.x | (bs.y << 16) | (kTerms ? bs.S << 24 : 0u);
   const int lane = threadIdx.x & 63, wave = threadIdx.x >> 6;
   const int c = lane & 31, h = lane >> 5;
   const float r2_hi = s->r2_hi, eps = s->screen_eps_m, S = s->mfma_scale, be = s->band_e;
@@ -851,7 +892,7 @@
 #endif
   const uint32_t sxy = kPlan ? slice_xy : 0u;
   const int64_t sxl = (int64_t)(sxy & 0xFFFFu);
-  const unsigned syl = sxy >> 16;
+  const unsigned syl = kTerms ? (sxy >> 16) & 0xFFu : sxy >> 16;
 #define M3D_NN_SX (kPlan ? sxl : (int64_t)blockIdx.x)
 #define M3D_NN_SY (kPlan ? syl : blockIdx.y)
 #pragma unroll
@@ -884,9 +925,19 @@
         rec[5] = atomicMax(&clk_slow, 0u);
         rec[6] = (unsigned long long)M3D_NN_SX | ((unsigned long long)M3D_NN_SY << 32) | ((unsigned long long)cur.ty << 48);
         rec[7] = clk2b;
+        if (!kTerms) rec[8] = rec[9] = 0;
       }
     }
   }
+#endif
+#if M3D_NN_TU_TERMS_KERNEL
+#if M3D_NN_CLOCK
+  if constexpr (kTerms)
+    nn_terms_handoff(static_cast<const NnTermsDev*>(td), s, (unsigned)sxl, sxy >> 24,
+                     blockIdx.x < kClkBlocks ? g_nn_clock + kClkWords * (int64_t)blockIdx.x : nullptr);
+#else
+  if constexpr (kTerms) nn_terms_handoff(static_cast<const NnTermsDev*>(td), s, (unsigned)sxl, sxy >> 24);
+#endif
 #endif
 }
 
@@ -919,6 +970,24 @@
   return per > 0 ? per : 1;
 }
 #endif
+hipError_t launch_nn_terms_kernel(unsigned blocks, hipStream_t st, M3D_NN_KERNEL_ARGS, NnPlan pl, const void* td);
+int nn_terms_kernel_blocks_per_cu();
+#if M3D_NN_TU_TERMS_KERNEL
+__global__ __launch_bounds__(kMBlock) __attribute__((amdgpu_waves_per_eu(4))) void nn_mfma_terms_kernel(
+    M3D_NN_KERNEL_ARGS, NnPlan pl, const NnTermsDev* __restrict__ td) {
+  nn_mfma_body<true, true>(src32, ns, tgt16, tgt32, tbox, nt_pad, off, s, keys, near2, sa, q0, pl, td);
+}
+hipError_t launch_nn_terms_kernel(unsigned blocks, hipStream_t st, M3D_NN_KERNEL_ARGS, NnPlan pl, const void* td) {
+  nn_mfma_terms_kernel<<<dim3(blocks), kMBlock, 0, st>>>(src32, ns, tgt16, tgt32, tbox, nt_pad, off, s, keys, near2, sa,
+                                                         q0, pl, static_cast<const NnTermsDev*>(td));
+  return hipGetLastError();
+}
+int nn_terms_kernel_blocks_per_cu() {
+  int per = 0;
+  if (hipOccupancyMaxActiveBlocksPerMultiprocessor(&per, nn_mfma_terms_kernel, kMBlock, 0) != hipSuccess) return 0;
+  return per > 0 ? per : 1;
+}
+#endif
 #undef M3D_NN_KERNEL_ARGS
 #if M3D_NN_TU_MAIN
 
@@ -959,20 +1028,43 @@
   return icp_nn_uses_mfma(s);
 }
 
+struct NnLaunchShape {
+  int64_t bx, gy;
+  bool planned;
+};
+static NnLaunchShape nn_launch_shape(const m3d_icp* s, int64_t q0, int64_t ns) {
+  const int64_t tt = (int64_t)kTH * kMTile;
+  const int64_t bx = (ns - q0 + kMQueries - 1) / kMQueries;
+  const int64_t gy = nn_grid_y(bx, s->tgrid->mf_npad / tt, nn_resident_slots(), M3D_NN_CULL != 0);
+  const bool planned = nn_plan_on() && s->nn_qblocks > 0 && q0 == 0 && ns == s->src->n && bx == s->nn_qblocks &&
+                       bx * gy <= s->nn_budget;
+  return NnLaunchShape{bx, gy, planned};
+}
+
+bool icp_nn_planned(const m3d_icp* s) {
+  if (s->src->n <= 0 || s->tgt->n == 0 || !icp_nn_uses_mfma(s) || s->tgrid->mf_npad % ((int64_t)kTH * kMTile) != 0)
+    return false;
+  return nn_launch_shape(s, 0, s->src->n).planned;
+}
+
 hipError_t launch_icp_nn(const m3d_icp* s, int64_t off, bool self_seed, hipStream_t st, int64_t q0,
-                         int64_t q1) {
+                         int64_t q1, bool with_terms) {
   const int64_t ns = q1 < 0 ? s->src->n : q1;
-  if (ns <= q0 || s->tgt->n == 0) return hipSuccess;
+  if (ns <= q0 || s->tgt->n == 0) return with_terms ? hipErrorInvalidValue : hipSuccess;
   const Grid* tg = s->tgrid;
   const int64_t tt = (int64_t)kTH * kMTile;
   if (!icp_nn_uses_mfma(s) || tg->mf_npad % tt != 0) return hipErrorInvalidValue;
-  const int64_t slots = nn_resident_slots();
-  const int64_t bx = (ns - q0 + kMQueries - 1) / kMQueries;
-  const int64_t gy = nn_grid_y(bx, tg->mf_npad / tt, slots, M3D_NN_CULL != 0);
+  const NnLaunchShape sh = nn_launch_shape(s, q0, ns);
+  const int64_t bx = sh.bx, gy = sh.gy;
   const bool by_rec = M3D_NN_SEED_REC != 0 && self_seed && off == 0 && s->tgt->rec64 != nullptr && s->seed != nullptr;
   const SeedArgs sa{s->corr, by_rec ? s->seed : s->tgt->xyz32, s->tgt->n, by_rec ? 2 : self_seed ? 1 : 0};
-  const bool planned = nn_plan_on() && s->nn_qblocks > 0 && q0 == 0 && ns == s->src->n && bx == s->nn_qblocks &&
-                       bx * gy <= s->nn_budget;
+  const bool planned = sh.planned;
+  if (with_terms) {
+    if (!planned || s->nn_targs == nullptr) return hipErrorInvalidValue;
+    return launch_nn_terms_kernel((unsigned)s->nn_budget, st, s->src->xyz32, ns, tg->mf16, tg->mf32, tg->mfbox,
+                                  tg->mf_npad, off, s->state, s->keys, s->near2, sa, q0,
+                                  NnPlan{s->nn_table, s->nn_cnt, (int)bx, (int)gy}, s->nn_targs);
+  }
   if (planned)
     return launch_nn_plan_kernel((unsigned)s->nn_budget, st, s->src->xyz32, ns, tg->mf16, tg->mf32, tg->mfbox,
                                  tg->mf_npad, off, s->state, s->keys, s->near2, sa, q0,
@@ -989,9 +1081,10 @@
     if (hipGetDevice(&dev) != hipSuccess || hipGetDeviceProperties(&p, dev) != hipSuccess) return (int64_t)0;
     if (hipOccupancyMaxActiveBlocksPerMultiprocessor(&per, nn_mfma_kernel, kMBlock, 0) != hipSuccess)
       return (int64_t)0;
-    const int pp = nn_plan_kernel_blocks_per_cu();
+    const int pp = nn_plan_kernel_blocks_per_cu(), pt = nn_terms_kernel_blocks_per_cu();
     per = per > 0 ? per : 1;
     if (pp > 0 && pp < per) per = pp;
+    if (pt > 0 && pt < per) per = pt;
     return (int64_t)p.multiProcessorCount * per;
   }();
   return slots;
diff --git a/3d-matching_amd/csrc/nn_brute_terms.hip b/3d-matching_amd/csrc/nn_brute_terms.hip
--- /dev/null
+++ b/3d-matching_amd/csrc/nn_brute_terms.hip
@@ -0,0 +1,2 @@
+#define M3D_NN_BRUTE_TERMS_TU 1
+#include "nn_brute.hip"
diff --git a/3d-matching_amd/m3d/_lib.py b/3d-matching_amd/m3d/_lib.py
--- a/3d-matching_amd/m3d/_lib.py
+++ b/3d-matching_amd/m3d/_lib.py
@@ -254,6 +254,9 @@
     "m3d_debug_icp_nn_plan": (C.c_int, [vp, vp, C.c_int64, vp]),
     "m3d_debug_icp_nn_plan_read": (C.c_int, [vp, vp, vp, vp, vp]),
     "m3d_debug_icp_seed_read": (C.c_int, [vp, vp, vp, vp, vp, vp]),
+    "m3d_debug_icp_nn_terms": (C.c_int, [vp, C.c_int]),
+    "m3d_debug_icp_nn_terms_read": (C.c_int, [vp, vp, vp, vp]),
+    "m3d_debug_nn_terms_select": (C.c_int, [C.c_uint32]),
     "m3d_parse_ascii_rows": (C.c_int, [C.c_char_p, C.c_size_t, i64, i32, C.POINTER(dbl),
                                        C.POINTER(C.c_size_t)]),
     "m3d_format_ascii_rows": (C.c_int, [C.POINTER(dbl), i64, i32, vp, C.c_size_t, C.POINTER(C.c_size_t)]),
diff --git a/include/m3d.h b/include/m3d.h
--- a/include/m3d.h
+++ b/include/m3d.h
@@ -442,6 +442,9 @@
 int m3d_debug_icp_nn_plan(m3d_icp* s, const int32_t* S, int64_t n, void* stream);
 int m3d_debug_icp_nn_plan_read(m3d_icp* s, uint32_t* counts, uint32_t* table, int32_t* shape3, void* stream);
 int m3d_debug_icp_seed_read(m3d_icp* s, float* seed, int32_t* corr, float* tgt32, int32_t* info2, void* stream);
+int m3d_debug_icp_nn_terms(m3d_icp* s, int on);
+int m3d_debug_icp_nn_terms_read(m3d_icp* s, uint32_t* tickets, uint32_t* counts, void* stream);
+int m3d_debug_nn_terms_select(uint32_t bits);
 
 
 int m3d_parse_ascii_rows(const char* buf, size_t len, int64_t rows, int32_t cols, double* out,
```

New measurement: 21500 ICP iter/s (100k src x 100k tgt per GPU) (median of 6 runs). 1.05x the previous value.
